# althonos/pyrodigal

Hardware: AMD Instinct MI355X
Metric: Mbp/sec gene-called (meta mode) (higher is better)
Workload: dtype f64; 1 GPU; 100000x20kbp_gc30-70_meta; contigs=100000, bases=2000000000, models=16, contigs_rank0=100000, sub_batch_contigs=6250, contexts_per_gpu=4, genes_all_ranks=2908995, steps_issued=a join of the contexts and a gather per step

## Files before the change

### pyrodigal_amd/csrc/finder.hip

```cpp
#include "pga_internal.h"
#include "pipeline.h"
#include "dpw_core.h"
#include "dev_common.h"

#include <math.h>
#include <stdio.h>
#include <stdlib.h>
#include <string.h>

#include <algorithm>
#include <atomic>
#include <chrono>
#include <condition_variable>
#include <functional>
#include <limits>
#include <map>
#include <memory>
#include <mutex>
#include <new>
#include <thread>
#include <unordered_map>

namespace {

// ... 322 lines not shown
        if (v.strand[ndx] == -1 && next_rev) ig = igm_same_h(v, ndx, next->stop_ndx, w);
        int mi[2] = {-1, -1}; double ms[2] = {0, 0}, mg[2] = {0, 0};
        const int sv_ndx = v.stop_val[ndx];
        constexpr int TWB = 40;
        for (int j0 = ndx - 100; j0 < ndx + 100; j0 += TWB) {
          unsigned long long pass = 0;
#pragma unroll
          for (int q = 0; q < TWB; q++) {
            const int j = j0 + q;
            const int jj = j < 0 ? 0 : (j >= nn ? nn - 1 : j);
            const bool ok = !(is_stop_n(v, jj) | (v.stop_val[jj] != sv_ndx)) && j >= 0 && j < nn && j != ndx;
            pass |= (unsigned long long)ok << q;
          }
          while (pass) {
            const int q = __builtin_ctzll(pass);
            pass &= pass - 1ull;
            const int j = j0 + q;
            double tg = 0.0;
            if (v.strand[j] == 1 && prev_fwd) {
                if (v.ndx[prev->stop_ndx] - v.ndx[j] > maxov) continue;
                tg = igm_same_h(v, prev->stop_ndx, j, w);
            }
            if (v.strand[j] == 1 && prev_rev) { if (v.ndx[prev->start_ndx] - v.ndx[j] >= 0) continue; tg = -0.15 * w; }
            if (v.strand[j] == -1 && next_fwd) { if (v.ndx[j] - v.ndx[next->start_ndx] >= 0) continue; tg = -0.15 * w; }
            if (v.strand[j] == -1 && next_rev) {
                if (v.ndx[j] - v.ndx[next->stop_ndx] > maxov) continue;
                tg = igm_same_h(v, j, next->stop_ndx, w);
            }
            const double cs = v.cscore[j] + v.sscore[j];
            if (mi[0] == -1) { mi[0] = j; ms[0] = cs; mg[0] = tg; }
            else if (cs + tg > ms[0]) { mi[1] = mi[0]; ms[1] = ms[0]; mg[1] = mg[0]; mi[0] = j; ms[0] = cs; mg[0] = tg; }
            else if (mi[1] == -1 || cs + tg > ms[1]) { mi[1] = j; ms[1] = cs; mg[1] = tg; }
          }
        }
        for (int k = 0; k < 2; k++) {
            const int m = mi[k];
            if (m == -1) continue;
            if (v.tscore[m] < v.tscore[ndx] && ms[k] - v.tscore[m] >= sc - v.tscore[ndx] + w && v.rscore[m] > v.rscore[ndx] &&
                v.uscore[m] > v.uscore[ndx] && v.cscore[m] > v.cscore[ndx] && abs(v.ndx[m] - v.ndx[ndx]) > 15) {
                ms[k] += v.tscore[ndx] - v.tscore[m];
            } else if (abs(v.ndx[m] - v.ndx[ndx]) <= 15 && v.rscore[m] + v.tscore[m] > v.rscore[ndx] + v.tscore[ndx] &&
                       v.edge[ndx] == 0 && v.edge[m] == 0) {
                if (v.cscore[ndx] > v.cscore[m]) ms[k] += v.cscore[ndx] - v.cscore[m];
                if (v.uscore[ndx] > v.uscore[m]) ms[k] += v.uscore[ndx] - v.uscore[m];
                if (ig > mg[k]) ms[k] += ig - mg[k];
            } else ms[k] = -1000.0;
        }
        int pick = -1;
        for (int k = 0; k < 2; k++) {
            if (mi[k] == -1) continue;
            if (pick == -1 && ms[k] + mg[k] > sc + ig) pick = k;
            else if (pick >= 0 && ms[k] + mg[k] > ms[pick] + mg[pick]) pick = k;
        }
        if (pick != -1 && v.strand[mi[pick]] == 1) { cur.start_ndx = mi[pick]; cur.begin = v.ndx[mi[pick]] + 1; }
        else if (pick != -1 && v.strand[mi[pick]] == -1) { cur.start_ndx = mi[pick]; cur.end = v.ndx[mi[pick]] + 1; }
    }
}

void tweak_final_starts(const NodeView& v, std::vector<GeneRec>& g, double w, int maxov, int inner_threads = 1, WorkerPool* pool = nullptr) {
    const int ng = (int)g.size();
    if (inner_threads <= 1 || ng < 2048 || pool == nullptr) {
        for (int i = 0; i < ng; i++) tweak_one(v, i > 0 ? &g[i - 1] : nullptr, g[i], i < ng - 1 ? &g[i + 1] : nullptr, w, maxov);
        return;
    }
    const std::vector<GeneRec> orig(g);
    std::atomic<int> next(0);
    auto work = [&]() {
        for (;;) {
            const int i0 = next.fetch_add(256);
            if (i0 >= ng) break;
            for (int i = i0; i < std::min(ng, i0 + 256); i++)
                tweak_one(v, i > 0 ? &orig[i - 1] : nullptr, g[i], i < ng - 1 ? &orig[i + 1] : nullptr, w, maxov);
        }
    };
    pool->run(work, inner_threads);
    for (int i = 1; i < ng; i++) {
        if (g[i - 1].start_ndx == orig[i - 1].start_ndx) continue;
        g[i] = orig[i];
        tweak_one(v, &g[i - 1], g[i], i < ng - 1 ? &orig[i + 1] : nullptr, w, maxov);
    }
}

struct OutArrays;
struct TailDesc {
    int64_t out_off;
    int64_t gene_off;
    int32_t n;
    int32_t mx;
    double  st_wt;
    int64_t fin_off, topo_off;
    int32_t group, _pad;
    int64_t dp_off;
};
struct WinDesc {
    int64_t out_off;
    int64_t dp_off;
    int64_t fin_off;
    int64_t topo_off;
    int32_t n;
    int32_t _pad;
};
struct GcPtrs { const float* p[4]; };
struct OutArrays {
    int32_t* ndx; int32_t* stop_val; uint8_t* type; int8_t* strand; float* gc_cont;
    uint8_t* edge_dp; double* cscore_dp; double* sscore_dp; double* rscore_dp; double* uscore_dp; double* tscore_dp;
    int32_t* star_ptr; int32_t* traceb; int8_t* ov_mark; double* score;
    uint8_t* edge; double* cscore; double* sscore; double* rscore; double* uscore; double* tscore; double* mot_score;
    int32_t* mot_ndx; uint8_t* rbs; uint8_t* mot_len; uint8_t* mot_spacer; uint8_t* mot_spacendx;
    int32_t direct;
    const int32_t* g_ndx[4]; const int32_t* g_stop_val[4]; const uint8_t* g_type[4]; const int8_t* g_strand[4];
    const uint8_t* c_edge; const double* c_cscore; const double* c_rscore; const double* c_uscore; const double* c_tscore;
    const int32_t* c_star_ptr; const double* d_score;
};

__global__ void __launch_bounds__(256)
k_gather_winners(const WinDesc* __restrict__ wd, int n_win, int64_t out_begin, int64_t total, GroupArrays ga, ChainArrays ca,
                 DpBuffers dp, OutArrays o, const int lean ) {
    __shared__ int s_w0;
    const int64_t blk0 = out_begin + (int64_t)blockIdx.x * blockDim.x;
    const int64_t g = blk0 + threadIdx.x;
    int lo = block_search_le([&](const int k) { return wd[k].out_off; }, n_win, blk0, &s_w0);
    if (g >= out_begin + total) return;
    while (lo + 1 < n_win && wd[lo + 1].out_off <= g) lo++;
    const WinDesc w = wd[lo];
    const int i = (int)(g - w.out_off);
    const int64_t t = w.topo_off + i, a = w.dp_off + i, f = w.fin_off + i;
    if (o.direct) { o.sscore_dp[g] = ca.sscore[a]; o.traceb[g] = dp.traceb[a]; o.ov_mark[g] = dp.ov_mark[a]; return; }
    o.ndx[g] = ga.ndx[t]; o.stop_val[g] = ga.stop_val[t]; o.type[g] = ga.type[t]; o.strand[g] = ga.strand[t];
    o.edge_dp[g] = ca.edge[a]; o.cscore_dp[g] = ca.cscore[a]; o.sscore_dp[g] = ca.sscore[a]; o.rscore_dp[g] = ca.rscore[a];
    o.uscore_dp[g] = ca.uscore[a]; o.tscore_dp[g] = ca.tscore[a];
    o.star_ptr[3 * g] = ca.star_ptr[3 * a]; o.star_ptr[3 * g + 1] = ca.star_ptr[3 * a + 1]; o.star_ptr[3 * g + 2] = ca.star_ptr[3 * a + 2];
    o.traceb[g] = dp.traceb[a]; o.ov_mark[g] = dp.ov_mark[a]; o.score[g] = dp.score[a];
    if (lean) return;
    o.gc_cont[g] = ga.gc_cont[t];
    o.edge[g] = ca.edge[f]; o.cscore[g] = ca.cscore[f]; o.sscore[g] = ca.sscore[f]; o.rscore[g] = ca.rscore[f];
    o.uscore[g] = ca.uscore[f]; o.tscore[g] = ca.tscore[f]; o.mot_score[g] = ca.mot_score[f]; o.mot_ndx[g] = ca.mot_ndx[f];
    o.rbs[2 * g] = ca.rbs[2 * f]; o.rbs[2 * g + 1] = ca.rbs[2 * f + 1];
    o.mot_len[g] = ca.mot_len[f]; o.mot_spacer[g] = ca.mot_spacer[f]; o.mot_spacendx[g] = ca.mot_spacendx[f];
}

struct GeneNodeAttr {
    double cscore, sscore, rscore, uscore, tscore, mot_score;
    float gc_cont; int32_t mot_ndx;
    uint8_t edge, rbs0, rbs1, mot_len, mot_spacer, _pad[3];
};
__global__ void __launch_bounds__(256)
k_gather_gene_nodes(const int64_t* __restrict__ idx, int n, OutArrays o, GeneNodeAttr* __restrict__ out) {
    const int t = blockIdx.x * blockDim.x + threadIdx.x;
    if (t >= n) return;
    const int64_t g = idx[t];
    GeneNodeAttr a;
    a.cscore = o.cscore[g]; a.sscore = o.sscore[g]; a.rscore = o.rscore[g]; a.uscore = o.uscore[g]; a.tscore = o.tscore[g];
    a.mot_score = o.mot_score[g]; a.gc_cont = o.gc_cont[g]; a.mot_ndx = o.mot_ndx[g];
    a.edge = o.edge[g]; a.rbs0 = o.rbs[2 * g]; a.rbs1 = o.rbs[2 * g + 1]; a.mot_len = o.mot_len[g]; a.mot_spacer = o.mot_spacer[g];
    a._pad[0] = a._pad[1] = a._pad[2] = 0;
    out[t] = a;
}

__device__ inline NodeView node_view(const TailDesc& d, const OutArrays& o, int32_t* tracef, uint8_t* elim) {
    const int64_t oo = d.out_off;
    if (o.direct) {
        const int64_t t = d.topo_off, a = d.dp_off; const int g = d.group;
        return NodeView{d.n, o.g_ndx[g] + t, o.g_stop_val[g] + t, o.g_type[g] + t, o.g_strand[g] + t, o.c_edge + a,
                        const_cast<double*>(o.c_cscore) + a, o.sscore_dp + oo, o.c_rscore + a, o.c_uscore + a, o.c_tscore + a,
                        o.c_star_ptr + 3 * a, o.traceb + oo, tracef + oo, o.ov_mark + oo, o.d_score + a, elim + oo};
    }
    return NodeView{d.n, o.ndx + oo, o.stop_val + oo, o.type + oo, o.strand + oo, o.edge_dp + oo,
                    o.cscore_dp + oo, o.sscore_dp + oo, o.rscore_dp + oo, o.uscore_dp + oo, o.tscore_dp + oo,
                    o.star_ptr + 3 * oo, o.traceb + oo, tracef + oo, o.ov_mark + oo, o.score + oo, elim + oo};
}

__global__ void __launch_bounds__(64)
k_tail_path(const TailDesc* __restrict__ td, int n_contigs, OutArrays o, int32_t* tracef, uint8_t* elim, int32_t* __restrict__ path,
            GeneRec* __restrict__ genes, int32_t* __restrict__ n_genes) {
    const int i = blockIdx.x * blockDim.x + threadIdx.x;
    if (i >= n_contigs) return;
// ... 159 lines not shown
                  const GeneRec* __restrict__ orig, GeneRec* __restrict__ out, const int32_t* __restrict__ n_genes, int maxov,
                  uint8_t* __restrict__ changed, int32_t* __restrict__ n_changed) {
    const int c = blockIdx.y, lane = threadIdx.x & 63;
    const int g = blockIdx.x * 4 + (threadIdx.x >> 6), ng = n_genes[c];
    if (g >= ng) return;
    const TailDesc d = td[c];
    const NodeView v = node_view(d, o, tracef, elim);
    const GeneRec* base = orig + d.gene_off;
    GeneRec cur = base[g];
    GeneRec prev{}, nxt{};
    if (g > 0) prev = base[g - 1];
    if (g < ng - 1) nxt = base[g + 1];
    tweak_one_wave(v, g > 0 ? &prev : nullptr, cur, g < ng - 1 ? &nxt : nullptr, d.st_wt, maxov, lane);
    if (lane != 0) return;
    out[d.gene_off + g] = cur;
    const bool moved = cur.start_ndx != base[g].start_ndx && v.strand[cur.start_ndx] == -1;
    changed[d.gene_off + g] = moved ? 1 : 0;
    if (moved) atomicAdd(&n_changed[c], 1);
}

#define PGA_FIX_MAXWIN 4096
__global__ void __launch_bounds__(1024)
k_tail_tweak_fixup(const TailDesc* __restrict__ td, int n_contigs, OutArrays o, int32_t* tracef, uint8_t* elim,
                   const GeneRec* __restrict__ orig, const GeneRec* __restrict__ par_all, const int32_t* __restrict__ n_genes, int maxov,
                   const uint8_t* __restrict__ ch0_all, const int32_t* __restrict__ n_changed, GeneRec* __restrict__ fin_all,
                   uint8_t* __restrict__ chf_all) {
    __shared__ uint8_t s_redone[PGA_FIX_MAXWIN];
    const int c = blockIdx.x, lane = threadIdx.x & 63, wave = threadIdx.x >> 6, nwaves = blockDim.x >> 6;
    if (c >= n_contigs) return;
    const TailDesc d = td[c];
    const int ng = n_genes[c];
    const GeneRec* ob = orig + d.gene_off; const GeneRec* par = par_all + d.gene_off; const uint8_t* ch0 = ch0_all + d.gene_off;
    GeneRec* fin = fin_all + d.gene_off; uint8_t* chf = chf_all + d.gene_off;
    for (int g = threadIdx.x; g < ng; g += blockDim.x) { fin[g] = par[g]; chf[g] = ch0[g]; }
    if (n_changed[c] == 0 || ng < 2) return;
    __threadfence_block();
    __syncthreads();
    const NodeView v = node_view(d, o, tracef, elim);
    const int nwin = (ng - 1 + 63) >> 6;
    auto run_window = [&](const int w, const bool assume) -> bool {
        const int g0 = 1 + (w << 6), g1 = min(ng, g0 + 64);
        const int g = g0 + lane;
        if (!assume) {
            if (g < g1) { fin[g] = par[g]; chf[g] = ch0[g]; }
            __builtin_amdgcn_fence(__ATOMIC_RELEASE, "workgroup");
            __builtin_amdgcn_fence(__ATOMIC_ACQUIRE, "workgroup");
        }
        const int pf = g < g1 ? ((lane == 0 && !assume) ? chf[g - 1] : ch0[g - 1]) : 0;
        unsigned long long mask = __ballot(pf != 0);
        bool last = false;
        while (mask) {
            const int k = __builtin_ctzll(mask);
            mask &= mask - 1ull;
            const int gg = g0 + k;
            GeneRec cur = ob[gg];
            const GeneRec prev = (k == 0 && assume) ? par[gg - 1] : fin[gg - 1];
            GeneRec nxt{};
            if (gg < ng - 1) nxt = ob[gg + 1];
            tweak_one_wave(v, &prev, cur, gg < ng - 1 ? &nxt : nullptr, d.st_wt, maxov, lane);
            const int nf = cur.start_ndx != ob[gg].start_ndx && v.strand[cur.start_ndx] == -1;
            if (lane == 0) { fin[gg] = cur; chf[gg] = (uint8_t)nf; }
            __builtin_amdgcn_fence(__ATOMIC_RELEASE, "workgroup");
            __builtin_amdgcn_fence(__ATOMIC_ACQUIRE, "workgroup");
            if (gg + 1 < g1) { if (nf) mask |= 1ull << (k + 1); else mask &= ~(1ull << (k + 1)); }
            if (gg == g1 - 1) last = true;
        }
        return last;
    };
    if (nwin <= PGA_FIX_MAXWIN) {
        for (int w = wave; w < nwin; w += nwaves) { const bool r = run_window(w, true); if (lane == 0) s_redone[w] = r; }
        __threadfence_block();
        __syncthreads();
        if (wave == 0)
            for (int w = 1; w < nwin; w++)
                if (s_redone[w - 1]) { const bool r = run_window(w, false); if (lane == 0) s_redone[w] = r; __builtin_amdgcn_wave_barrier(); }
    } else if (wave == 0) {
        for (int w = 0; w < nwin; w++) run_window(w, false);
    }
}

__global__ void __launch_bounds__(256)
k_emit_genes(const TailDesc* __restrict__ td, int n_contigs, int64_t n_slots, OutArrays o, const GeneRec* __restrict__ fin,
             const int32_t* __restrict__ n_genes, const int64_t* __restrict__ gene_begin, int single, pga_gene* __restrict__ out,
             const int lean, ChainArrays ca, GcPtrs gcs) {
    const int64_t slot = (int64_t)blockIdx.x * blockDim.x + threadIdx.x;
    if (slot >= n_slots) return;
    const int c = contig_of_slot(td, n_contigs, slot);
    const TailDesc d = td[c];
    const int g = (int)(slot - d.gene_off);
    if (g >= n_genes[c]) return;
    const GeneRec gr = fin[slot];
    const int64_t sn = d.out_off + gr.start_ndx, en = d.out_off + gr.stop_ndx;
    pga_gene G;
    memset(&G, 0, sizeof G);
    G.contig = c; G.begin = gr.begin; G.end = gr.end; G.start_ndx = gr.start_ndx; G.stop_ndx = gr.stop_ndx;
    if (o.direct) {
        const int64_t ts = d.topo_off + gr.start_ndx, as = d.dp_off + gr.start_ndx, ae = d.dp_off + gr.stop_ndx;
        const int64_t fs = d.fin_off + gr.start_ndx, fe = d.fin_off + gr.stop_ndx;
        G.strand = o.g_strand[d.group][ts];
        const uint8_t se = single ? o.c_edge[as] : ca.edge[fs], ee = single ? o.c_edge[ae] : ca.edge[fe];
        G.partial_begin = G.strand == 1 ? se : ee; G.partial_end = G.strand == 1 ? ee : se;
        G.start_type = se ? 3 : o.g_type[d.group][ts];
        G.rbs[0] = ca.rbs[2 * fs]; G.rbs[1] = ca.rbs[2 * fs + 1];
        G.mot_len = ca.mot_len[fs]; G.mot_spacer = ca.mot_spacer[fs]; G.mot_ndx = ca.mot_ndx[fs]; G.mot_score = ca.mot_score[fs];
        G.gc_cont = gcs.p[d.group][ts];
        G.cscore = single ? o.c_cscore[as] : ca.cscore[fs]; G.sscore = single ? o.sscore_dp[sn] : ca.sscore[fs];
        G.rscore = single ? o.c_rscore[as] : ca.rscore[fs]; G.uscore = single ? o.c_uscore[as] : ca.uscore[fs];
        G.tscore = single ? o.c_tscore[as] : ca.tscore[fs];
        out[gene_begin[c] + g] = G;
        return;
    }
    G.strand = o.strand[sn];
    if (lean) {
        const int64_t fs = d.fin_off + gr.start_ndx, fe = d.fin_off + gr.stop_ndx;
        const uint8_t se = single ? o.edge_dp[sn] : ca.edge[fs], ee = single ? o.edge_dp[en] : ca.edge[fe];
        G.partial_begin = G.strand == 1 ? se : ee; G.partial_end = G.strand == 1 ? ee : se;
        G.start_type = se ? 3 : o.type[sn];
        G.rbs[0] = ca.rbs[2 * fs]; G.rbs[1] = ca.rbs[2 * fs + 1];
        G.mot_len = ca.mot_len[fs]; G.mot_spacer = ca.mot_spacer[fs]; G.mot_ndx = ca.mot_ndx[fs]; G.mot_score = ca.mot_score[fs];
        G.gc_cont = gcs.p[d.group][d.topo_off + gr.start_ndx];
        G.cscore = single ? o.cscore_dp[sn] : ca.cscore[fs]; G.sscore = single ? o.sscore_dp[sn] : ca.sscore[fs];
        G.rscore = single ? o.rscore_dp[sn] : ca.rscore[fs]; G.uscore = single ? o.uscore_dp[sn] : ca.uscore[fs];
        G.tscore = single ? o.tscore_dp[sn] : ca.tscore[fs];
        out[gene_begin[c] + g] = G;
        return;
    }
    const uint8_t se = single ? o.edge_dp[sn] : o.edge[sn], ee = single ? o.edge_dp[en] : o.edge[en];
    G.partial_begin = G.strand == 1 ? se : ee; G.partial_end = G.strand == 1 ? ee : se;
    G.start_type = se ? 3 : o.type[sn];
    G.rbs[0] = o.rbs[2 * sn]; G.rbs[1] = o.rbs[2 * sn + 1];
    G.mot_len = o.mot_len[sn]; G.mot_spacer = o.mot_spacer[sn]; G.mot_ndx = o.mot_ndx[sn]; G.mot_score = o.mot_score[sn];
    G.gc_cont = o.gc_cont[sn];
    G.cscore = single ? o.cscore_dp[sn] : o.cscore[sn]; G.sscore = single ? o.sscore_dp[sn] : o.sscore[sn];
    G.rscore = single ? o.rscore_dp[sn] : o.rscore[sn]; G.uscore = single ? o.uscore_dp[sn] : o.uscore[sn];
    G.tscore = single ? o.tscore_dp[sn] : o.tscore[sn];
    out[gene_begin[c] + g] = G;
}

__global__ void __launch_bounds__(256)
k_cover_genes(const pga_gene* __restrict__ genes, int64_t n_genes, const ContigDesc* __restrict__ ct, int n_contigs, uint32_t* __restrict__ bits) {
    const int64_t g = (int64_t)blockIdx.x * 4 + (threadIdx.x >> 6);
    const int lane = threadIdx.x & 63;
    if (g >= n_genes) return;
    const int c = genes[g].contig;
    if (c < 0 || c >= n_contigs) return;
    const int32_t b = max(genes[g].begin, 1), e = min(genes[g].end, ct[c].len);
    if (b > e) return;
    const int64_t b0 = ct[c].base + b - 1, b1 = ct[c].base + e - 1;
    const int64_t w0 = b0 >> 5, w1 = b1 >> 5;
    for (int64_t w = w0 + lane; w <= w1; w += 64) {
        uint32_t m = 0xffffffffu;
        if (w == w0) m &= 0xffffffffu << (b0 & 31);
        if (w == w1) m &= 0xffffffffu >> (31 - (b1 & 31));
        atomicOr(&bits[w], m);
    }
}

__global__ void __launch_bounds__(256)
k_count_cover(const uint32_t* __restrict__ bits, const ContigDesc* __restrict__ ct, int64_t* __restrict__ coding) {
    __shared__ int64_t part[4];
    const int c = blockIdx.x;
    const int64_t lo = ct[c].base, len = ct[c].len;
    int64_t n = 0;
    if (len > 0) {
        const int64_t hi = lo + len - 1, w0 = lo >> 5, w1 = hi >> 5;
        for (int64_t w = w0 + threadIdx.x; w <= w1; w += blockDim.x) {
            uint32_t m = bits[w];
            if (w == w0) m &= 0xffffffffu << (lo & 31);
            if (w == w1) m &= 0xffffffffu >> (31 - (hi & 31));
            n += __popc(m);
        }
    }
    for (int d = 32; d > 0; d >>= 1) n += __shfl_down(n, d, 64);
    if ((threadIdx.x & 63) == 0) part[threadIdx.x >> 6] = n;
    __syncthreads();
    if (threadIdx.x == 0) coding[c] = part[0] + part[1] + part[2] + part[3];
}

#include "tail.inl"

struct ResultOwner {
    pga_result pub;
    std::vector<pga_contig_result> contigs;
    std::vector<pga_gene> genes;
    pga_gene* pin_genes = nullptr; size_t pin_cap = 0, pin_n = 0;
    std::vector<pga_nodes> nodes;
    std::vector<int32_t> mask_off, masks;
    bool has_masks = false;
// ... 478 lines not shown
        return PGA_EINVAL;
    }
    const int32_t n_contigs = batch->n;
    if (!c->finder) { int rc0 = pga_finder_models_changed(c); if (rc0) return rc0; }
    const bool meta_run = pp->meta && stage == 0;
    const bool use_sets = meta_run && !batch->sets.empty();
    const bool per_contig = model_of_contig != nullptr && !pp->meta && stage != PGA_STAGE_EXTRACT && stage != PGA_STAGE_SEQUENCE;
    const bool per_contig_tt = tt_of_contig != nullptr && stage == PGA_STAGE_EXTRACT;
    if (c->n_models <= 0 && !meta_run && stage != PGA_STAGE_EXTRACT && stage != PGA_STAGE_SEQUENCE) { c->err = "pga_find_genes: no model loaded (call pga_set_models first)"; return PGA_EINVAL; }
    const pga_params P = *pp;
    const bool mask_union = batch->mask_case != 0 || !batch->regions.empty();
    if ((P.mask || batch->mask_case) && P.min_mask < 0) { c->err = "pga_find_genes: min_mask must be positive"; return PGA_EINVAL; }
    if (!P.closed && P.min_edge_gene > 0 && P.min_edge_gene < 4) {
        c->err = "pga_find_genes: min_edge_gene below 4 is not supported with open ends";
        return PGA_EINVAL;
    }
    if (P.min_gene <= 0 || P.min_edge_gene <= 0 || P.max_overlap < 0 || P.max_overlap > P.min_gene) {
        c->err = "pga_find_genes: invalid min_gene / min_edge_gene / max_overlap";
        return PGA_EINVAL;
    }
    HT(c, hipSetDevice(c->device));
    FinderState* f = c->finder;
    hipStream_t st = c->stream;
    const bool multi = per_contig || per_contig_tt;
    std::vector<int> cgrp, gtt;
    if (per_contig) {
        gtt = f->group_tt;
        for (int i = 0; i < n_contigs; i++) cgrp.push_back(f->model_group[model_of_contig[i]]);
    } else if (per_contig_tt) {
        for (int i = 0; i < n_contigs; i++) {
            int g = (int)(std::find(gtt.begin(), gtt.end(), tt_of_contig[i]) - gtt.begin());
            if (g == (int)gtt.size()) gtt.push_back(tt_of_contig[i]);
            cgrp.push_back(g);
        }
    }
    const int NC = n_contigs, NM = c->n_models, NG = meta_run ? (int)f->group_tt.size() : (multi ? std::max(1, (int)gtt.size()) : 1);
    if (NG > 4) { c->err = "pga_find_genes: more than 4 distinct translation tables loaded"; return PGA_EINVAL; }
    if (const char* fault = getenv("PGA_FAULT_CONTIG_LEN")) {
        const long fl = atol(fault);
        for (int i = 0; i < NC; i++) if ((long)batch->ct[i].len == fl) { c->err = "pga_find_genes: fault injected by PGA_FAULT_CONTIG_LEN"; return PGA_EDEVICE; }
    }

    std::vector<int32_t> set_of;
    int NS = 0;
    if (use_sets) {
        set_of.resize((size_t)NC);
        std::unordered_map<int32_t, int32_t> dense;
        for (int i = 0; i < NC; i++) {
            const int32_t lab = batch->sets[(size_t)i];
            if (lab < 0) { set_of[(size_t)i] = NS++; continue; }
            auto it = dense.find(lab);
            if (it == dense.end()) it = dense.emplace(lab, NS++).first;
            set_of[(size_t)i] = it->second;
        }
        c->set_model.assign((size_t)NC, -1);
        c->set_score.assign((size_t)NC, std::numeric_limits<double>::quiet_NaN());
        c->model_scores.assign((size_t)NC * (size_t)NM, std::numeric_limits<double>::quiet_NaN());
        c->model_scores_nm = NM;
    }

    ResultOwner* R = new (std::nothrow) ResultOwner();
    if (!R) return PGA_ENOMEM;
    struct Guard { ResultOwner* r; ~Guard() { delete r; } } guard{R};
    R->contigs.assign(NC, pga_contig_result{-1, 0, 0, 0, 0, 0.0, 0.0});
    R->mask_off.assign(NC + 1, 0);
    R->has_masks = P.mask || mask_union;
    memset(&R->pub, 0, sizeof R->pub);
    R->pub.n_contigs = NC;

    const std::vector<ContigDesc>& ct = batch->ct;
    const int64_t total = batch->total;
    StageTimer tm;

    if (NC > 0 && total > 0) {
        const char* d_seq = batch->d_seq;
        DEVBUF(d_dig, uint8_t, "d_dig", total + 16);
        DEVBUF(d_ct, ContigDesc, "d_ct", NC + 1);
        const size_t xa_cnt = 4, xa_cbase = xa_cnt + 2 * (size_t)NC, xa_sbase = xa_cbase + (size_t)NG * (NC + 1), xa_en = xa_sbase + (size_t)NG * (NC + 1);
        const size_t xa_words = xa_en + ((size_t)NG * NC + 3) / 4 + 1;
        DEVBUF(d_xa, int32_t, "d_extract_info", xa_words);
        PINBUF(h_xa, int32_t, "h_extract_info", xa_words);
        int32_t* const d_st_overflow = d_xa; int32_t* const h_st_overflow = h_xa;
        int32_t* const d_cnt = d_xa + xa_cnt; int32_t* const h_cnt = h_xa + xa_cnt;
        const int64_t gc_blocks = pga_gc_blocks(total);
        DEVBUF(d_p16, int32_t, "d_gc_p16", total / 16 + 2);
        DEVBUF(d_gc_bsum, int32_t, "d_gc_bsum", gc_blocks + 1);
        DEVBUF(d_gc_boff, int32_t, "d_gc_boff", gc_blocks + 1);
        int32_t* const d_cbase = d_xa + xa_cbase; int32_t* const h_cbase = h_xa + xa_cbase;
        DEVBUF(d_tile_first, int32_t, "d_tile_first", (size_t)6 * batch->n_tiles);
        DEVBUF(d_tile_last, int32_t, "d_tile_last", (size_t)6 * batch->n_tiles);
        DEVBUF(d_tile_count, int32_t, "d_tile_count", (size_t)NG * (batch->n_tiles + 1));
        DEVBUF(d_tile_off, int32_t, "d_tile_off", (size_t)NG * (batch->n_tiles + 1));
        DEVBUF(d_tile_scount, int32_t, "d_tile_scount", (size_t)NG * (batch->n_tiles + 1));
        DEVBUF(d_tile_soff, int32_t, "d_tile_soff", (size_t)NG * (batch->n_tiles + 1));
        int32_t* const d_sbase = d_xa + xa_sbase; int32_t* const h_sbase = h_xa + xa_sbase;
        uint8_t* const d_enabled = (uint8_t*)(d_xa + xa_en); uint8_t* const h_enabled = (uint8_t*)(h_xa + xa_en);

        GroupArrays ga[4];
        for (int g = 0; g < NG; g++) {
            char nm[32];
#define GBUF(field, type, count) { snprintf(nm, sizeof nm, #field "%d", g); void* p__; int rc__ = ensure_dev(c, nm, sizeof(type) * (size_t)(count) + 64, &p__); if (rc__) return rc__; ga[g].field = (type*)p__; }
            GBUF(df, uint8_t, total + 16)
            GBUF(c16, int32_t, (size_t)batch->n_tiles * 192 + 2)
            ga[g].tile0 = batch->d_tile0;
            ga[g].ndx = nullptr; ga[g].stop_val = nullptr; ga[g].type = nullptr; ga[g].strand = nullptr; ga[g].edge0 = nullptr; ga[g].gc_cont = nullptr;
        }

        HT(c, hipEventRecord(f->e_start, st));
        HT(c, hipMemcpyAsync(d_ct, ct.data(), sizeof(ContigDesc) * (NC + 1), hipMemcpyHostToDevice, st));
        HT(c, hipMemsetAsync(d_xa, 0, sizeof(int32_t) * xa_cbase, st));
        pga_launch_digitize(d_seq, d_dig, total, d_ct, NC, d_cnt, d_cnt + NC, st);
        pga_launch_gc_prefix(d_dig, total, d_gc_bsum, d_gc_boff, d_p16, st);
        MaskList masks{nullptr, nullptr};
        int32_t* h_moff = nullptr; const int2* d_union_iv = nullptr;
        if (mask_union) {
            const int64_t per_source = total / std::max(1, P.min_mask) + NC + 1;
            const int64_t most = std::min<int64_t>((P.mask ? per_source : 0) + (batch->mask_case ? per_source : 0) + (int64_t)batch->regions.size(),
                                                   total / 2 + NC + 1);
            const int cap = (int)std::min<int64_t>(most, (int64_t)1 << 28);
            DEVBUF(d_bits, uint32_t, "d_mask_bits", 2 * pga_mask_words(total) + 2);
            DEVBUF(d_mcounts, int32_t, "d_mask_counts", 4 * (pga_mask_waves(total) + 1));
            DEVBUF(d_moff, int32_t, "d_mask_off", NC + 2);
            DEVBUF(d_miv, int2, "d_mask_iv", cap + 1);
            PINBUF(h_moff_, int32_t, "h_mask_off", NC + 2);
            pga_launch_mask_union(d_dig, d_seq, total, d_ct, NC, batch->d_tiles, batch->n_tiles, P.mask, batch->mask_case, P.min_mask, batch->d_regions,
                                  (int)batch->regions.size(), d_bits, d_mcounts, d_moff, d_miv, cap, st);
            HT(c, hipMemcpyAsync(h_moff_, d_moff, sizeof(int32_t) * (NC + 1), hipMemcpyDeviceToHost, st));
            h_moff = h_moff_; d_union_iv = d_miv;
            masks = MaskList{d_moff, d_miv};
        } else if (P.mask) {
            const int cap = (int)std::min<int64_t>(total / std::max(1, P.min_mask) + NC + 1, (int64_t)1 << 28);
            DEVBUF(d_runs, MaskRun, "d_mask_runs", cap + 1);
            DEVBUF(d_nruns, int32_t, "d_mask_count", 4);
            DEVBUF(d_moff, int32_t, "d_mask_off", NC + 2);
            DEVBUF(d_miv, int2, "d_mask_iv", cap + 1);
            pga_launch_find_masks(d_dig, d_ct, NC, batch->d_tiles, batch->n_tiles, P.min_mask, d_runs, d_nruns, cap, st);
            int32_t nruns = 0;
            HT(c, hipMemcpyAsync(&nruns, d_nruns, 4, hipMemcpyDeviceToHost, st));
            HT(c, hipStreamSynchronize(st));
            nruns = std::min(nruns, cap);
            std::vector<MaskRun> runs((size_t)nruns);
            if (nruns > 0) HT(c, hipMemcpy(runs.data(), d_runs, sizeof(MaskRun) * nruns, hipMemcpyDeviceToHost));
            std::sort(runs.begin(), runs.end(), [](const MaskRun& a, const MaskRun& b) { return a.contig != b.contig ? a.contig < b.contig : a.begin < b.begin; });
            std::vector<int32_t> moff(NC + 1, 0);
            std::vector<int2> miv((size_t)nruns + 1);
            for (int k = 0; k < nruns; k++) { moff[runs[k].contig + 1]++; miv[k] = make_int2(runs[k].begin, runs[k].end); }
            for (int i = 0; i < NC; i++) moff[i + 1] += moff[i];
            R->mask_off = moff;
            R->masks.resize(2 * (size_t)nruns);
            for (int k = 0; k < nruns; k++) { R->masks[2 * k] = runs[k].begin; R->masks[2 * k + 1] = runs[k].end; }
            HT(c, hipMemcpy(d_moff, moff.data(), sizeof(int32_t) * (NC + 1), hipMemcpyHostToDevice));
            if (nruns > 0) HT(c, hipMemcpy(d_miv, miv.data(), sizeof(int2) * nruns, hipMemcpyHostToDevice));
            masks = MaskList{d_moff, d_miv};
        }
        if (stage == PGA_STAGE_SEQUENCE) {
            HT(c, hipMemcpyAsync(h_cnt, d_cnt, sizeof(int32_t) * 2 * (size_t)NC, hipMemcpyDeviceToHost, st));
            HT(c, hipGetLastError());
            HT(c, hipStreamSynchronize(st));
            for (int i = 0; i < NC; i++) {
                R->contigs[i].gc = ct[i].len > 0 ? (double)h_cnt[i] / (double)ct[i].len : 0.0;
                R->contigs[i].n_unknown = h_cnt[NC + i];
            }
            if (h_moff) { const int rc = fetch_mask_union(c, R, h_moff, d_union_iv, NC); if (rc) return rc; }
            return publish(R, guard.r, P, out);
        }
        if (meta_run && NM > 0 && use_sets) {
            DEVBUF(d_set_of, int32_t, "d_set_of", 3 * (size_t)NC + 1);
            HT(c, hipMemcpyAsync(d_set_of, set_of.data(), sizeof(int32_t) * (size_t)NC, hipMemcpyHostToDevice, st));
            pga_launch_group_enable_sets(d_ct, NC, d_cnt, d_set_of, d_set_of + NC, f->d_model_gc, f->d_model_grp, NM, NG, d_enabled, st);
        } else if (meta_run && NM > 0) {
            pga_launch_group_enable(d_ct, NC, d_cnt, f->d_model_gc, f->d_model_grp, NM, NG, d_enabled, st);
        }
        if (multi) {
            for (int g = 0; g < NG; g++) for (int i = 0; i < NC; i++) h_enabled[(size_t)g * NC + i] = cgrp[i] == g;
            HT(c, hipMemcpyAsync(d_enabled, h_enabled, (size_t)NG * NC, hipMemcpyHostToDevice, st));
        }
        if (getenv("PGA_STAGE_FULL")) f->stage_full = true;
        bool stage_full = f->stage_full;
        c->extract_passes = 0;
        for (;;) {
            const bool half = !stage_full;
            const int shift = half ? std::max(1, std::min(8, getenv("PGA_STAGE_SHIFT") ? atoi(getenv("PGA_STAGE_SHIFT")) : 1)) : 0;
            const int64_t st_slots = half ? (total >> shift) + (int64_t)PGA_STAGE_SLACK * batch->n_tiles + 8 : 2 * total + 2;
            for (int g = 0; g < NG; g++) {
                char nm[32];
                GBUF(st_ndx, int32_t, st_slots) GBUF(st_sv, int32_t, st_slots) GBUF(st_info, uint8_t, st_slots)
                ga[g].st_half = shift; ga[g].st_overflow = d_st_overflow;
            }
            if (c->extract_passes > 0) HT(c, hipMemsetAsync(d_st_overflow, 0, sizeof(int32_t), st));
            for (int g = 0; g < NG; g++) {
                const int tt = meta_run ? f->group_tt[g] : multi ? gtt[g] : (stage == PGA_STAGE_EXTRACT ? tt_override : c->models[0].trans_table);
                pga_launch_extract(d_dig, total, d_ct, NC, tt, P, ga[g], batch->d_tiles, batch->n_tiles, batch->d_tile0, d_tile_first, d_tile_last,
                                   d_tile_count + (size_t)g * (batch->n_tiles + 1), d_tile_off + (size_t)g * (batch->n_tiles + 1), d_cbase + (size_t)g * (NC + 1),
                                   d_tile_scount + (size_t)g * (batch->n_tiles + 1), d_tile_soff + (size_t)g * (batch->n_tiles + 1), d_sbase + (size_t)g * (NC + 1),
                                   masks, st, ((meta_run && NM > 0) || multi) ? d_enabled + (size_t)g * NC : nullptr);
            }
            HT(c, hipMemcpyAsync(h_xa, d_xa, sizeof(int32_t) * xa_words, hipMemcpyDeviceToHost, st));
            HT(c, hipGetLastError());
            HT(c, hipStreamSynchronize(st));
            c->extract_passes++;
            if (!half || h_st_overflow[0] == 0) break;
            stage_full = true;
            if (!getenv("PGA_STAGE_SHIFT")) f->stage_full = true;
        }
        if (h_moff) { const int rc = fetch_mask_union(c, R, h_moff, d_union_iv, NC); if (rc) return rc; }

        tm.mark("extract+sync");
        int64_t group_nodes[4] = {0, 0, 0, 0};
        for (int g = 0; g < NG; g++) {
            char nm[32];
            group_nodes[g] = h_cbase[(size_t)g * (NC + 1) + NC];
            const int64_t n = group_nodes[g] + 1;
            GBUF(ndx, int32_t, n) GBUF(stop_val, int32_t, n) GBUF(type, uint8_t, n) GBUF(strand, int8_t, n) GBUF(edge0, uint8_t, n) GBUF(gc_cont, float, n) GBUF(contig_of, int32_t, n)
            GBUF(stop_list, int32_t, (int64_t)h_sbase[(size_t)g * (NC + 1) + NC] + 1)
            GBUF(start_list, int32_t, group_nodes[g] - (int64_t)h_sbase[(size_t)g * (NC + 1) + NC] + 1)
            GBUF(ovl_topo, uint32_t, (int64_t)h_sbase[(size_t)g * (NC + 1) + NC] + 1)
            GBUF(srank, int32_t, n + 4)
        }
        for (int g = 0; g < NG; g++) {
            pga_launch_place(d_ct, batch->d_tiles, batch->n_tiles, d_tile_off + (size_t)g * (batch->n_tiles + 1),
                             d_tile_soff + (size_t)g * (batch->n_tiles + 1), ga[g], st);
            pga_launch_orf_gc(d_ct, NC, d_dig, d_p16, ga[g], (int)group_nodes[g], d_cbase + (size_t)g * (NC + 1), st);
        }
        std::vector<std::vector<ChainDesc>> gch(NG);
        std::vector<double> mgc((size_t)NM); std::vector<int> mtt((size_t)NM);
        for (int m = 0; m < NM; m++) { mgc[m] = c->models[m].gc; mtt[m] = c->models[m].trans_table; }
        for (int g = 0; g < NG; g++) gch[g].reserve(meta_run ? (size_t)NC * 6 : (size_t)NC);
        std::vector<double> set_gc;
        if (use_sets) {
            std::vector<int64_t> sum((size_t)2 * NS, 0);
            for (int i = 0; i < NC; i++) { sum[2 * (size_t)set_of[i]] += h_cnt[i]; sum[2 * (size_t)set_of[i] + 1] += ct[i].len; }
            set_gc.resize((size_t)NS);
            for (int s = 0; s < NS; s++) set_gc[(size_t)s] = sum[2 * (size_t)s + 1] > 0 ? (double)sum[2 * (size_t)s] / (double)sum[2 * (size_t)s + 1] : 0.0;
        }
        for (int i = 0; i < NC; i++) {
            const int L = ct[i].len;
            double gc = L > 0 ? (double)h_cnt[i] / (double)L : 0.0;
            R->contigs[i].gc = gc;
            R->contigs[i].n_unknown = h_cnt[NC + i];
            if (!meta_run) {
                const int m = per_contig ? model_of_contig[i] : 0, g = multi ? cgrp[i] : 0;
                const int32_t* cb = h_cbase + (size_t)g * (NC + 1);
                ChainDesc ch{0, cb[i], cb[i + 1] - cb[i], m, i, 1};
                ch.group = g;
                gch[g].push_back(ch);
                continue;
            }
            if (use_sets) gc = set_gc[(size_t)set_of[i]];
            const double low = fmin(0.65, 0.88495 * gc - 0.0102337), high = fmax(0.35, 0.86596 * gc + 0.1131991);
            int tt_prev = -1;
            for (int m = 0; m < NM; m++) {
                if (mgc[m] < low || mgc[m] > high) continue;
                const int g = f->model_group[m];
                if (!h_enabled[(size_t)g * NC + i]) { c->err = "pga_find_genes: host and device disagree on a GC window"; return PGA_EDEVICE; }
                const int32_t* cb = h_cbase + (size_t)g * (NC + 1);
                ChainDesc ch{0, cb[i], cb[i + 1] - cb[i], m, i, mtt[m] != tt_prev ? 1 : 0};
                ch.group = g;
                tt_prev = mtt[m];
                gch[g].push_back(ch);
            }
        }
        std::vector<ChainDesc> chains;
        { size_t tot = 0; for (int g = 0; g < NG; g++) tot += gch[g].size(); chains.reserve(tot); }
        std::vector<int> g_c0(NG + 1, 0);
        std::vector<int64_t> g_n0(NG + 1, 0);
        int64_t tot_chain_nodes = 0, tot_chain_stops = 0;
        std::vector<int64_t> g_s0(NG + 1, 0);
        for (int g = 0; g < NG; g++) {
            g_c0[g] = (int)chains.size(); g_n0[g] = tot_chain_nodes;
            for (ChainDesc& ch : gch[g]) {
                ch.off = tot_chain_nodes; tot_chain_nodes += ch.n;
                ch.soff = tot_chain_stops;
                const int32_t* sb = h_sbase + (size_t)ch.group * (NC + 1);
                tot_chain_stops += sb[ch.contig + 1] - sb[ch.contig];
                chains.push_back(ch);
            }
            g_s0[g + 1] = tot_chain_stops;
        }
        g_c0[NG] = (int)chains.size(); g_n0[NG] = tot_chain_nodes;
        const int NCH = (int)chains.size();
        R->pub.node_passes = tot_chain_nodes;
        R->pub.n_chains = NCH;
        int64_t max_rescore = 0;
        if (meta_run) for (int g = 0; g < NG; g++) max_rescore += h_cbase[(size_t)g * (NC + 1) + NC];
        const int64_t chain_cap = tot_chain_nodes + max_rescore + 64;

        ChainArrays ca;
        {
            DEVBUF(a0, double, "ca_cscore", chain_cap) DEVBUF(a1, double, "ca_sscore", chain_cap) DEVBUF(a2, double, "ca_rscore", chain_cap)
            DEVBUF(a3, double, "ca_uscore", chain_cap) DEVBUF(a4, double, "ca_tscore", chain_cap) DEVBUF(a5, double, "ca_mot_score", chain_cap)
            DEVBUF(a6, int32_t, "ca_star_ptr", 3 * chain_cap) DEVBUF(a7, int32_t, "ca_mot_ndx", chain_cap) DEVBUF(a8, uint8_t, "ca_rbs", 2 * chain_cap)
            DEVBUF(a9, uint8_t, "ca_edge", chain_cap) DEVBUF(a10, uint8_t, "ca_mot_len", chain_cap) DEVBUF(a11, uint8_t, "ca_mot_spacer", chain_cap)
            DEVBUF(a12, uint8_t, "ca_mot_spacendx", chain_cap)
            int64_t max_contig_nodes = 0;
            for (int g = 0; g < NG; g++) for (int i = 0; i < NC; i++)
                max_contig_nodes = std::max<int64_t>(max_contig_nodes, h_cbase[(size_t)g * (NC + 1) + i + 1] - h_cbase[(size_t)g * (NC + 1) + i]);
            DEVBUF(a13, double, "ca_cscore_raw", chain_cap + max_contig_nodes + 64)
            ca = ChainArrays{a0, a1, a2, a3, a4, a5, a13, a6, a7, a8, a9, a10, a11, a12, a13 + chain_cap};
        }
        DpSegPlan seg_plan;
        const bool use_wave = stage == 0 && pga_dp_use_wave(NCH);
        bool seg_wave = false;
        if (stage == 0 && !use_wave && pga_dpw_use_sched() && !getenv("PGA_DP_KERNEL")) {
            int64_t cand = 0;
            const int min_chain = std::max(256, getenv("PGA_DP_SEG_MIN") ? atoi(getenv("PGA_DP_SEG_MIN")) : 16384);
            for (int k = 0; k < NCH; k++) if (chains[(size_t)k].n >= min_chain) cand += chains[(size_t)k].n;
            const char* e = getenv("PGA_DP_SEG_WAVE");
            const char* m = getenv("PGA_DP_SEG_WAVE_MIN");
            seg_wave = e ? atoi(e) != 0 : cand >= (m ? atoll(m) : 2500000ll);
        }
        bool wave_prep = use_wave || seg_wave;
        bool use_sched = wave_prep && pga_dpw_use_sched();
        std::vector<int32_t> h_bbase;
        if (use_sched) {
            h_bbase.resize((size_t)NG * (NC + 1));
            for (int g = 0; g < NG; g++) {
                const int32_t* cb = h_cbase + (size_t)g * (NC + 1);
                int32_t* bb = h_bbase.data() + (size_t)g * (NC + 1);
                bb[0] = 0;
                for (int i = 0; i < NC; i++) bb[i + 1] = bb[i] + ((cb[i + 1] - cb[i] + 63) >> 6);
            }
            for (ChainDesc& ch : chains) ch.sched_b0 = h_bbase[(size_t)ch.group * (NC + 1) + ch.contig];
        }
        int max_batches[4] = {0, 0, 0, 0};
        if (use_sched) for (int g = 0; g < NG; g++) for (int i = 0; i < NC; i++)
            max_batches[g] = std::max(max_batches[g], h_bbase[(size_t)g * (NC + 1) + i + 1] - h_bbase[(size_t)g * (NC + 1) + i]);
        bool segmented = stage == 0 && !use_wave && pga_dp_plan(chains.data(), NCH, tot_chain_nodes, seg_plan, seg_wave);
        if (seg_wave && !segmented) { seg_wave = false; wave_prep = use_wave; use_sched = false; h_bbase.clear(); }
        const bool lean_gather = !P.want_nodes && !(getenv("PGA_TAIL") && strcmp(getenv("PGA_TAIL"), "host") == 0) && !getenv("PGA_FULL_GATHER");
        const bool direct_gather = lean_gather && !getenv("PGA_GATHER_ALL_DP");
        const int64_t dp_cap = tot_chain_nodes + seg_plan.extra + 1;
        const int64_t dp_slots = NCH + (int64_t)seg_plan.segs.size() + 1;
        const int64_t tree_cap = use_wave ? 1 : (seg_wave ? tot_chain_nodes + 1 : dp_cap);
        DpBuffers dp;
        {
            DEVBUF(b0, DpSrc, "dp_src", tree_cap) DEVBUF(b1, DpTgt, "dp_tgt", tree_cap)
            DEVBUF(b2, double, "dp_score", dp_cap) DEVBUF(b3, int32_t, "dp_traceb", dp_cap)
            DEVBUF(b4, int32_t, "dp_tbn", dp_cap) DEVBUF(b5, int8_t, "dp_ov", dp_cap)
            DEVBUF(b7, double, "dp_chain_results", 2 * dp_slots + 2)
            int32_t* const b6 = (int32_t*)(b7 + dp_slots); int32_t* const b8 = b6 + dp_slots;
            DEVBUF(b9, double, "dp_A", tree_cap) DEVBUF(b10, double, "dp_V0", tree_cap) DEVBUF(b11, double, "dp_V1", tree_cap)
            DEVBUF(b12, double, "dp_V2", tree_cap) DEVBUF(b13, double, "dp_hv", tree_cap) DEVBUF(b14, int32_t, "dp_hi", tree_cap)
            dp = DpBuffers{b0, b1, b2, b3, b4, b5, b6, b7, b8, b9, {b10, b11, b12}, b13, b14, nullptr};
        }
        DpwGroupPtrs wgroups{};
        DpwBuffers wbuf{};
        if (wave_prep) {
            for (int g = 0; g < NG; g++) {
                char nm[32];
                const int64_t n = group_nodes[g] + 1;
#define WBUF(field, type) { snprintf(nm, sizeof nm, "dpw_" #field "%d", g); void* p__; int rc__ = ensure_dev(c, nm, sizeof(type) * (size_t)n + 64, &p__); if (rc__) return rc__; wgroups.g[g].field = (type*)p__; }
                WBUF(kf, uint8_t) WBUF(lo, int32_t) WBUF(q1, int32_t) WBUF(q2, int32_t)
#undef WBUF
                wgroups.g[g].ndx = ga[g].ndx; wgroups.g[g].stop_val = ga[g].stop_val; wgroups.g[g].srank = ga[g].srank;
                if (use_sched) {
                    const int64_t nbat = h_bbase[(size_t)g * (NC + 1) + NC];
                    void* p__; int rc__;
                    snprintf(nm, sizeof nm, "dpw_shdr%d", g); rc__ = ensure_dev(c, nm, sizeof(DpwSchedHdr) * (size_t)(nbat + 1), &p__); if (rc__) return rc__; wgroups.g[g].shdr = (DpwSchedHdr*)p__;
                    snprintf(nm, sizeof nm, "dpw_sent%d", g); rc__ = ensure_dev(c, nm, sizeof(DpwSlot) * (size_t)DPW_SCHED_STRIDE * (size_t)(nbat + 1) + 256, &p__); if (rc__) return rc__; wgroups.g[g].sent = (uint4*)p__;
                    snprintf(nm, sizeof nm, "dpw_scur%d", g); rc__ = ensure_dev(c, nm, 64, &p__); if (rc__) return rc__; wgroups.g[g].scur = (uint32_t*)p__;
                }
            }
            DEVBUF(w0, double, "dpw_cs", dp_cap + 2) DEVBUF(w1, DpwExt, "dpw_ext", tot_chain_stops + 4)       DEVBUF(w2, double, "dpw_sfxv", dp_cap) DEVBUF(w3, int32_t, "dpw_sfxi", dp_cap)
            wbuf = DpwBuffers{w0, w1, w2, w3};
            for (int g = 0; g < NG; g++) {
                if (g_c0[g + 1] - g_c0[g] == 0 || g_n0[g + 1] - g_n0[g] == 0 || stage == PGA_STAGE_EXTRACT) continue;
                int max_nodes_g = 0;
                for (int i = 0; i < NC; i++) max_nodes_g = std::max(max_nodes_g, h_cbase[(size_t)g * (NC + 1) + i + 1] - h_cbase[(size_t)g * (NC + 1) + i]);
                if (g < 4) HT(c, hipEventRecord(f->e_aux[4 * g], st));
                pga_launch_dpw_topo(wgroups.g[g], ga[g].type, ga[g].strand, d_cbase + (size_t)g * (NC + 1), NC, (int)group_nodes[g], st, max_nodes_g);
                if (g < 4) HT(c, hipEventRecord(f->e_aux[4 * g + 1], st));
            }
        }
        DpSegDev seg_dev{};
        if (segmented) {
            DEVBUF(seg_arena, char, "dp_seg_arena", pga_dp_seg_bytes(seg_plan, NCH, tot_chain_nodes));
            HT(c, pga_dp_seg_bind(seg_plan, NCH, tot_chain_nodes, seg_arena, st, &seg_dev));
            if (seg_wave) { seg_dev.wave_groups = &wgroups; seg_dev.wave_buf = &wbuf; }
        }
        int32_t* d_dp_order = nullptr;
        std::vector<int32_t> dp_order;
        if (use_wave && NCH > 1 && !getenv("PGA_DP_NO_ORDER")) {
            std::vector<int32_t> lens((size_t)NCH);
            for (int k = 0; k < NCH; k++) lens[(size_t)k] = chains[k].n;
            dp_order.resize((size_t)NCH);
            pga_dp_start_order(NCH, lens.data(), dp_order.data());
            static std::atomic<int> xcc_of[64];
            int n_xcc = xcc_of[c->device & 63].load();
            if (n_xcc == 0) {
                int v = 0;
                n_xcc = (hipDeviceGetAttribute(&v, hipDeviceAttributeNumberOfXccs, c->device) == hipSuccess && v > 0) ? v : 8;
                xcc_of[c->device & 63].store(n_xcc);
            }
            if (!(getenv("PGA_DP_XCD") && atoi(getenv("PGA_DP_XCD")) == 0) && NCH >= 64 && n_xcc == 8) {
                std::vector<int32_t> key((size_t)NCH), by_xcd((size_t)NCH * 8);
                for (int k = 0; k < NCH; k++) key[(size_t)k] = chains[(size_t)k].group * NC + chains[(size_t)k].contig;
                const int64_t nb = pga_dp_xcd_order(NCH, dp_order.data(), lens.data(), key.data(), NC * NG, by_xcd.data(), (int64_t)by_xcd.size());
                int64_t load[8] = {0, 0, 0, 0, 0, 0, 0, 0}, total = 0, heaviest = 0;
                for (int64_t k = 0; k < nb; k++) if (by_xcd[(size_t)k] >= 0) { load[k & 7] += lens[(size_t)by_xcd[(size_t)k]]; total += lens[(size_t)by_xcd[(size_t)k]]; }
                for (int q = 0; q < 8; q++) heaviest = std::max(heaviest, load[q]);
                if (nb > 0 && heaviest * 8 <= total + total * 3 / 10) { by_xcd.resize((size_t)nb); dp_order.swap(by_xcd); }
            }
        }
        PINBUF(h_maxscore, double, "h_chain_results", 2 * dp_slots + 2);
        int32_t* const h_maxidx = (int32_t*)(h_maxscore + dp_slots); int32_t* const h_ipath = h_maxidx + dp_slots;
        PINBUF(h_scur, uint32_t, "h_dpw_scur", 16);
        std::vector<int64_t> ovl_blk0((size_t)NG + 1, 0);
        for (int g = 0; g < NG; g++) ovl_blk0[(size_t)g + 1] = ovl_blk0[(size_t)g] + (g_s0[g + 1] - g_s0[g] + 255) / 256;
        const size_t pa_conv = 0, pa_cc = (((size_t)NG * NC + 1) + 7) & ~(size_t)7, pa_bb = pa_cc + sizeof(int2) * (size_t)2 * NG * NC,
                     pa_ord = pa_bb + ((sizeof(int32_t) * (h_bbase.size() + 1) + 7) & ~(size_t)7),
                     pa_blk = pa_ord + ((sizeof(int32_t) * (dp_order.size() + 1) + 7) & ~(size_t)7),
                     pa_ch = pa_blk + ((sizeof(int32_t) * ((size_t)ovl_blk0[NG] + 1) + 7) & ~(size_t)7), pa_copy = pa_ch + sizeof(ChainDesc) * (size_t)NCH;
        DEVBUF(d_plan, char, "d_call_plan", pa_copy + sizeof(ChainDesc) * ((size_t)NC + 2));
        PINBUF(h_plan, char, "h_call_plan", pa_copy + 64);
        uint8_t* const d_conv = (uint8_t*)(d_plan + pa_conv);
        int2* const d_cc = (int2*)(d_plan + pa_cc); int2* const h_cc = (int2*)(h_plan + pa_cc);
        int32_t* const d_bbase = use_sched ? (int32_t*)(d_plan + pa_bb) : nullptr;
        if (!dp_order.empty()) d_dp_order = (int32_t*)(d_plan + pa_ord);
        ChainDesc* const d_chains = (ChainDesc*)(d_plan + pa_ch);
        memset(h_plan + pa_conv, 0, pa_cc);
        for (size_t k = 0; k < (size_t)2 * NG * NC; k++) h_cc[k] = make_int2(0, 0);
        for (int k = 0; k < NCH; k++) {
            const int g = chains[k].group;
            int2& e = h_cc[(size_t)g * NC + chains[k].contig];
            if (e.y == 0) e.x = k;
            e.y++;
        }
        if (use_sched && !h_bbase.empty()) memcpy(h_plan + pa_bb, h_bbase.data(), sizeof(int32_t) * h_bbase.size());
        if (!dp_order.empty()) memcpy(h_plan + pa_ord, dp_order.data(), sizeof(int32_t) * dp_order.size());
        if (NCH > 0) memcpy(h_plan + pa_ch, chains.data(), sizeof(ChainDesc) * (size_t)NCH);
        const int32_t* const d_ovl_blk = (const int32_t*)(d_plan + pa_blk);
        {
            int32_t* const h_blk = (int32_t*)(h_plan + pa_blk);
            for (int g = 0; g < NG; g++) {
                int k = g_c0[g];
                const int64_t nb = ovl_blk0[(size_t)g + 1] - ovl_blk0[(size_t)g];
                for (int64_t b = 0; b < nb; b++) {
                    const int64_t p0 = g_s0[g] + 256 * b;
                    while (k + 1 < g_c0[g + 1] && chains[(size_t)k + 1].soff <= p0) k++;
                    h_blk[ovl_blk0[(size_t)g] + b] = k - g_c0[g];
                }
            }
        }
        HT(c, hipMemcpyAsync(d_plan, h_plan, pa_copy, hipMemcpyHostToDevice, st));

        tm.mark("plan+alloc");
        std::vector<int32_t> cs_tk[4], cs_en[4];
        ScoreParams sp{P.closed, P.meta, P.max_overlap, NM, nullptr, nullptr};
        PINBUF(h_conv, uint8_t, "h_conv_flag", (size_t)NG * NC + 1);
        const pga_training* d_models = (const pga_training*)c->d_models_raw;
        for (int g = 0; g < NG; g++) {
            const int nch = g_c0[g + 1] - g_c0[g];
            const int64_t nn = g_n0[g + 1] - g_n0[g];
            if (nch == 0 || nn == 0 || stage == PGA_STAGE_EXTRACT) continue;
            const void* d_cs_tasks = nullptr; const void* d_cs_entries = nullptr; int n_cs_tasks = 0;
            const char* cs_env = getenv("PGA_CS_LDS");
            const char* cs_tn = getenv("PGA_CS_TASK_NODES");
            const int cs_task_nodes = cs_tn && atoi(cs_tn) >= 256 && atoi(cs_tn) <= 8192 ? atoi(cs_tn) : 5120;
            if (!(cs_env && atoi(cs_env) == 0) && !f->gil_stride.empty()) {
                std::vector<int32_t>& tk = cs_tk[g]; std::vector<int32_t>& en = cs_en[g];
                if (pga_cs_tasks(h_cc + (size_t)g * NC, NC, chains.data(), h_cbase + (size_t)g * (NC + 1), f->model_rank.data(), cs_task_nodes, tk, en) && !tk.empty()) {
                    char nm1[32], nm2[32];
                    snprintf(nm1, sizeof nm1, "cs_tasks%d", g); snprintf(nm2, sizeof nm2, "cs_entries%d", g);
                    void* p1; void* p2;
                    { int rc__ = ensure_dev(c, nm1, tk.size() * 4 + 64, &p1); if (rc__) return rc__; }
                    { int rc__ = ensure_dev(c, nm2, en.size() * 4 + 64, &p2); if (rc__) return rc__; }
                    HT(c, hipMemcpyAsync(p1, tk.data(), tk.size() * 4, hipMemcpyHostToDevice, st));
                    HT(c, hipMemcpyAsync(p2, en.data(), en.size() * 4, hipMemcpyHostToDevice, st));
                    d_cs_tasks = p1; d_cs_entries = p2; n_cs_tasks = (int)(tk.size() / 4);
                }
            }
            sp.conv_flag = meta_run ? d_conv + (size_t)g * NC : nullptr;
            StopLaunch sl;
            sl.sbase = d_sbase + (size_t)g * (NC + 1); sl.soff_begin = g_s0[g]; sl.n_pairs = g_s0[g + 1] - g_s0[g];
            sl.n_stops = h_sbase[(size_t)g * (NC + 1) + NC];
            sl.starts_only = stage == 0 && !(getenv("PGA_SS_STARTS_ONLY") && atoi(getenv("PGA_SS_STARTS_ONLY")) == 0);
            sl.n_starts = (int32_t)(group_nodes[g] - sl.n_stops);
            sl.blk_chain = d_ovl_blk + ovl_blk0[(size_t)g];
            if (sl.starts_only && sl.n_starts > 0 && NM > 1 && !(getenv("PGA_SS_MM") && atoi(getenv("PGA_SS_MM")) == 0)) {
                std::vector<int64_t> mm_items;
                sl.mm_tiles = pga_mm_tiles(chains.data() + g_c0[g], nch, h_cbase + (size_t)g * (NC + 1), h_sbase + (size_t)g * (NC + 1), NM, mm_items);
                char nm[32];
                void* p__;
                snprintf(nm, sizeof nm, "ss_rec%d", g);
                { int rc__ = ensure_dev(c, nm, PGA_SS_REC_BYTES * (size_t)sl.n_starts + 64, &p__); if (rc__) return rc__; sl.mm_rec = p__; }
                snprintf(nm, sizeof nm, "ss_mmchain%d", g);
                { int rc__ = ensure_dev(c, nm, PGA_SS_MMCHAIN_BYTES * (size_t)nch + 64, &p__); if (rc__) return rc__; sl.mm_chain = p__; }
                snprintf(nm, sizeof nm, "ss_mmtile%d", g);
                { int rc__ = ensure_dev(c, nm, PGA_SS_MMTILE_BYTES * (size_t)sl.mm_tiles + 64, &p__); if (rc__) return rc__; sl.mm_tile = p__; }
                snprintf(nm, sizeof nm, "ss_mmscratch%d", g);
                { int rc__ = ensure_dev(c, nm, pga_mm_scratch_bytes(NM, nch), &p__); if (rc__) return rc__; sl.mm_scratch = p__; }
            }
            sp.cs_out = nullptr;
            if (wave_prep) {
                sl.topo_q2 = wgroups.g[g].q2; sl.ext = wbuf.ext; sp.cs_out = wbuf.cs;
                if (use_wave) {
                    sl.fill_star_ptr = !(stage == 0 && direct_gather);
                    sp.lean_stops = (stage == 0 && direct_gather && sl.starts_only && !getenv("PGA_SS_FULL_STOPS")) ? 1 : 0;
                }
            }
            pga_launch_score(d_chains + g_c0[g], nch, g_n0[g], nn, d_dig, d_ct, ga[g], d_models, f->d_msc, c->d_model_const, ca, sp,
                             d_chains, d_cc + (size_t)g * NC, d_cbase + (size_t)g * (NC + 1), NC, (int)group_nodes[g], f->d_sd_lut, st, 0,
                             (meta_run || per_contig || n_cs_tasks > 0) ? f->d_gil + f->gil_off[g] : nullptr, (meta_run || per_contig || n_cs_tasks > 0) ? f->gil_stride[g] : 0, f->d_model_rank,
                             d_cs_tasks, n_cs_tasks, d_cs_entries, &sl);
            if (wave_prep && use_sched) {
                if (g < 4) HT(c, hipEventRecord(f->e_aux[4 * g + 2], st));
                pga_launch_dpw_sched(wgroups.g[g], d_cbase + (size_t)g * (NC + 1), d_bbase + (size_t)g * (NC + 1), NC, max_batches[g], st);
                if (g < 4) HT(c, hipEventRecord(f->e_aux[4 * g + 3], st));
                HT(c, hipMemcpyAsync(h_scur + 2 * g, wgroups.g[g].scur, 2 * sizeof(uint32_t), hipMemcpyDeviceToHost, st));
            }
            NodeArrays na{ga[g].ndx, ga[g].stop_val, ga[g].type, ga[g].strand, ca.cscore, ca.sscore, ca.rscore, ca.uscore, ca.star_ptr};
            if (!use_wave && stage == 0) pga_launch_dp_prepare(d_chains + g_c0[g], nch, g_n0[g], nn, na, c->d_model_const, dp, st);
        }
        if (stage != 0) {
            const int64_t nn = tot_chain_nodes;
            PINBUF(hs_i32, int32_t, "hs_i32", 6 * nn + 8);
            PINBUF(hs_f64, double, "hs_f64", 6 * nn + 8);
            PINBUF(hs_u8, uint8_t, "hs_u8", 10 * nn + 8);
            PINBUF(hs_f32, float, "hs_f32", nn + 8);
            const bool scored = stage >= PGA_STAGE_SCORE;
            for (int g = 0; g < NG; g++) {
                const int64_t gn = group_nodes[g], o = g_n0[g];
                if (gn == 0) continue;
                HT(c, hipMemcpyAsync(hs_i32 + o, ga[g].ndx, 4 * gn, hipMemcpyDeviceToHost, st));
                HT(c, hipMemcpyAsync(hs_i32 + nn + o, ga[g].stop_val, 4 * gn, hipMemcpyDeviceToHost, st));
                HT(c, hipMemcpyAsync(hs_u8 + o, ga[g].type, gn, hipMemcpyDeviceToHost, st));
                HT(c, hipMemcpyAsync(hs_u8 + nn + o, ga[g].strand, gn, hipMemcpyDeviceToHost, st));
                if (!scored) HT(c, hipMemcpyAsync(hs_u8 + 2 * nn + o, ga[g].edge0, gn, hipMemcpyDeviceToHost, st));
                if (scored) HT(c, hipMemcpyAsync(hs_f32 + o, ga[g].gc_cont, 4 * gn, hipMemcpyDeviceToHost, st));
            }
            if (nn > 0) {
// ... 315 lines not shown
                ngenes += cr.n_genes;
                if (k < 0) { cr.model = -1; continue; }
                cr.model = chains[k].model; cr.n_nodes = chains[k].n;
                cr.score = P.meta ? 0.0 : (h_ipath[k] >= 0 ? h_maxscore[k] : 0.0);
            }
            R->genes.resize((size_t)ngenes);
            PINBUF(h_gidx, int64_t, "h_gidx", 2 * ngenes + 1);
            PINBUF(h_attr, GeneNodeAttr, "h_attr", 2 * ngenes + 1);
            if (ngenes > 0) {
                DEVBUF(d_gidx, int64_t, "d_gidx", 2 * ngenes + 1);
                DEVBUF(d_attr, GeneNodeAttr, "d_attr", 2 * ngenes + 1);
                for (int i = 0; i < NC; i++) {
                    int64_t gi = R->contigs[i].gene_begin;
                    for (const GeneRec& gr : cg[i]) { h_gidx[2 * gi] = out_off[i] + gr.start_ndx; h_gidx[2 * gi + 1] = out_off[i] + gr.stop_ndx; gi++; }
                }
                HT(c, hipMemcpyAsync(d_gidx, h_gidx, sizeof(int64_t) * 2 * ngenes, hipMemcpyHostToDevice, st));
                hipLaunchKernelGGL(k_gather_gene_nodes, dim3((unsigned)((2 * ngenes + 255) / 256)), dim3(256), 0, st, d_gidx, (int)(2 * ngenes), o, d_attr);
                HT(c, hipMemcpyAsync(h_attr, d_attr, sizeof(GeneNodeAttr) * 2 * ngenes, hipMemcpyDeviceToHost, st));
                HT(c, hipGetLastError());
                HT(c, hipStreamSynchronize(st));
            }
            tm.mark("gene_attrs");
            std::atomic<int> next2(0);
            auto filler = [&]() {
                for (;;) {
                    const int i = next2.fetch_add(1);
                    if (i >= NC) break;
                    const int k = win_chain[i];
                    if (k < 0) continue;
                    const int64_t oo = out_off[i];
                    const bool single = !P.meta;
                    int64_t gi = R->contigs[i].gene_begin;
                    for (const GeneRec& gr : cg[i]) {
                        pga_gene& G = R->genes[(size_t)gi];
                        const GeneNodeAttr& as = h_attr[2 * gi]; const GeneNodeAttr& ae = h_attr[2 * gi + 1];
                        gi++;
                        memset(&G, 0, sizeof G);
                        const int64_t sn = oo + gr.start_ndx, en = oo + gr.stop_ndx;
                        G.contig = i; G.begin = gr.begin; G.end = gr.end; G.start_ndx = gr.start_ndx; G.stop_ndx = gr.stop_ndx;
                        G.strand = h.strand[sn];
                        const uint8_t se = single ? h.edge_dp[sn] : as.edge, ee = single ? h.edge_dp[en] : ae.edge;
                        G.partial_begin = G.strand == 1 ? se : ee; G.partial_end = G.strand == 1 ? ee : se;
                        G.start_type = se ? 3 : h.type[sn];
                        G.rbs[0] = as.rbs0; G.rbs[1] = as.rbs1;
                        G.mot_len = as.mot_len; G.mot_spacer = as.mot_spacer; G.mot_ndx = as.mot_ndx; G.mot_score = as.mot_score;
                        G.gc_cont = as.gc_cont;
                        G.cscore = single ? h.cscore_dp[sn] : as.cscore; G.sscore = single ? h.sscore_dp[sn] : as.sscore;
                        G.rscore = single ? h.rscore_dp[sn] : as.rscore; G.uscore = single ? h.uscore_dp[sn] : as.uscore;
                        G.tscore = single ? h.tscore_dp[sn] : as.tscore;
                    }
                }
            };
            run_parallel(filler);
            if (coding) {
                std::vector<std::pair<int32_t, int32_t>> iv;
                for (int i = 0; i < NC; i++) {
                    iv.clear();
                    const int32_t len = ct[i].len;
                    for (const GeneRec& gr : cg[i]) {
                        const int32_t b = std::max<int32_t>(gr.begin, 1), e = std::min<int32_t>(gr.end, len);
                        if (b <= e) iv.emplace_back(b, e);
                    }
                    std::sort(iv.begin(), iv.end());
                    int64_t n = 0; int32_t hi = 0;
                    for (const auto& x : iv) {
                        if (x.second <= hi) continue;
                        n += x.second - std::max(x.first - 1, hi);
                        hi = x.second;
                    }
                    coding[i] = n;
                }
            }
        } else {
            tm.mark("gather");
            std::vector<TailDesc> tdv(NC);
            int64_t n_slots = 0;
            for (int i = 0; i < NC; i++) {
                const int k = win_chain[i];
                TailDesc& d = tdv[i];
                d.out_off = k >= 0 ? out_off[i] : 0; d.gene_off = n_slots;
                d.n = k >= 0 ? chains[k].n : 0; d.mx = k >= 0 ? h_maxidx[k] : -1;
                d.st_wt = k >= 0 ? c->models[chains[k].model].st_wt : 0.0;
                d.fin_off = k >= 0 ? fin_off[i] : 0; d.topo_off = k >= 0 ? chains[k].topo_off : 0;
                d.group = k >= 0 ? chains[k].group : 0; d._pad = 0;
                d.dp_off = k >= 0 ? chains[k].off : 0;
                n_slots += d.n / 2 + 2;
            }
            DEVBUF(d_td, TailDesc, "d_taildesc", NC + 1);
            DEVBUF(d_tracef, int32_t, "d_tracef", out_nodes + 1);
            DEVBUF(d_elim, uint8_t, "d_elim", out_nodes + 1);
            DEVBUF(d_gene0, GeneRec, "d_gene0", n_slots + 1);
            DEVBUF(d_gene1, GeneRec, "d_gene1", n_slots + 1);
            DEVBUF(d_ngenes, int32_t, "d_ngenes", NC + 1);
            DEVBUF(d_gbegin, int64_t, "d_gbegin", NC + 1);
            PINBUF(h_ngenes, int32_t, "h_ngenes", NC + 1);
            PINBUF(h_gbegin, int64_t, "h_gbegin", NC + 1);
            HT(c, hipMemcpyAsync(d_td, tdv.data(), sizeof(TailDesc) * NC, hipMemcpyHostToDevice, st));
            DEVBUF(d_path, int32_t, "d_path", out_nodes + 1);
            DEVBUF(d_changed, uint8_t, "d_changed", n_slots + 1);
            DEVBUF(d_nchanged, int32_t, "d_nchanged", NC + 1);
            const unsigned init_blocks = (unsigned)std::min<int64_t>(2048, (std::max<int64_t>(out_nodes, NC) + 256) / 256);
            if (!par_tail) {
                hipLaunchKernelGGL(k_tail_init, dim3(init_blocks), dim3(256), 0, st, d_tracef, d_elim, out_nodes, d_nchanged, (int32_t*)nullptr, NC, (int32_t*)nullptr, 0);
                hipLaunchKernelGGL(k_tail_path, dim3((NC + 63) / 64), dim3(64), 0, st, d_td, NC, o, d_tracef, d_elim, d_path, d_gene0, d_ngenes);
            } else {
                std::vector<TpSeg> segs;
                bool tail_inited = false;
                for (int i = 0; i < NC; i++) if (win_chain[i] >= 0 && chains[win_chain[i]].n > 0) segs.push_back(TpSeg{out_off[i], chains[win_chain[i]].n, i});
                std::sort(segs.begin(), segs.end(), [](const TpSeg& a, const TpSeg& b) { return a.off < b.off; });
                if (!segs.empty() && out_nodes > 0) {
                    if (out_nodes >= (1ll << 30)) { c->err = "pga_find_genes: more than 2^30 nodes in the winning chains of one batch"; return PGA_EINVAL; }
                    int levels = 1;
                    while ((1ll << levels) < max_n) levels++;
                    const unsigned nblk = (unsigned)((out_nodes + 255) / 256);
                    const bool tp_steps = getenv("PGA_TP_STEPS") != nullptr;
                    const bool tp_one = max_n <= TP_SMALL_MAX && !tp_steps;
                    const int64_t tpn = tp_one ? 0 : out_nodes;
                    DEVBUF(tp_seg, TpSeg, "tp_seg", segs.size()) DEVBUF(tp_up, int32_t, "tp_up", (size_t)2 * tpn)
                    DEVBUF(tp_mark, uint8_t, "tp_mark", tpn) DEVBUF(tp_slots, int32_t, "tp_slots", tpn)
                    DEVBUF(tp_ins, int32_t, "tp_ins", 2 * tpn) DEVBUF(tp_excl, int32_t, "tp_excl", tpn + 1)
                    DEVBUF(tp_bsum, int32_t, "tp_bsum", nblk + 1) DEVBUF(tp_cnt, int32_t, "tp_cnt", segs.size())
                    HT(c, hipMemcpyAsync(tp_seg, segs.data(), sizeof(TpSeg) * segs.size(), hipMemcpyHostToDevice, st));
                    hipLaunchKernelGGL(k_tail_init, dim3(init_blocks), dim3(256), 0, st, d_tracef, d_elim, out_nodes, d_nchanged, d_ngenes, NC,
                                       tp_one ? (int32_t*)nullptr : tp_cnt, (int)segs.size());
                    tail_inited = true;
                    const TpWork tw{tp_seg, (int)segs.size(), out_nodes, levels, tp_up, tp_mark, tp_slots, tp_ins, tp_excl, tp_bsum, tp_cnt};
                    const dim3 grid(nblk), blk(256);
                    if (tp_one) {
                        const int cap = (int)((max_n + 63) & ~63ll);
                        hipLaunchKernelGGL(k_tp_small, dim3((unsigned)segs.size()), dim3(max_n <= 2048 ? 64 : 256), sizeof(int32_t) * 3 * (size_t)cap, st, tw, d_td, o,
                                           d_tracef, d_elim, d_gene0, d_ngenes, cap);
                    } else {
                    hipLaunchKernelGGL(k_tp_init, grid, blk, 0, st, tw, d_td, o);
                    {
                        const bool j8 = !(getenv("PGA_TP_JUMP8") && atoi(getenv("PGA_TP_JUMP8")) == 0);
                        int k = 0;
                        for (int left = levels; left > 0; k++) {
                            const int32_t* in = tp_up + (size_t)(k & 1) * out_nodes; int32_t* outp = tp_up + (size_t)((k + 1) & 1) * out_nodes;
                            if (j8 && left >= 3) { hipLaunchKernelGGL(k_tp_jump8, grid, blk, 0, st, tw, in, outp); left -= 3; }
                            else { hipLaunchKernelGGL(k_tp_jump, grid, blk, 0, st, tw, in, outp); left -= 1; }
                        }
                    }
                    hipLaunchKernelGGL(k_tp_slots, grid, blk, 0, st, tw, d_td, o);
                    hipLaunchKernelGGL(k_tp_scan1, grid, blk, 0, st, tw);
                    hipLaunchKernelGGL(k_tp_scan2, dim3(1), dim3(1024), 0, st, tw, (int)nblk);
                    hipLaunchKernelGGL(k_tp_scan3, grid, blk, 0, st, tw);
                    hipLaunchKernelGGL(k_tp_fill, grid, blk, 0, st, tw, o, d_path);
                    hipLaunchKernelGGL(k_tp_link, grid, blk, 0, st, tw, o, d_path, d_tracef);
                    hipLaunchKernelGGL(k_tp_elim_a, grid, blk, 0, st, tw, d_td, o, d_path);
                    hipLaunchKernelGGL(k_tp_elim_b, grid, blk, 0, st, tw, d_td, o, d_path, d_elim);
                    if (max_n >= 32768 && segs.size() <= 64 && !getenv("PGA_TP_EXTRACT_ONE")) {
                        const int chunks = (max_n + 1023) / 1024;
                        DEVBUF(tp_xsum, TpChunkSum, "tp_xsum", (size_t)chunks * segs.size() + 1);
                        const dim3 xg((unsigned)chunks, (unsigned)segs.size());
                        hipLaunchKernelGGL(k_tp_extract_sum, xg, dim3(1024), 0, st, tw, d_td, o, d_path, d_elim, tp_xsum, chunks);
                        hipLaunchKernelGGL(k_tp_extract_chunk, xg, dim3(1024), 0, st, tw, d_td, o, d_path, d_elim, (const TpChunkSum*)tp_xsum, chunks, d_gene0,
                                           d_ngenes);
                    } else
                    hipLaunchKernelGGL(k_tp_extract, dim3((unsigned)segs.size()), dim3(max_n >= 32768 ? 1024 : 256), 0, st, tw, d_td, o, d_path, d_elim,
                                       d_gene0, d_ngenes);
                    }
                }
                if (!tail_inited) hipLaunchKernelGGL(k_tail_init, dim3(init_blocks), dim3(256), 0, st, d_tracef, d_elim, out_nodes, d_nchanged, d_ngenes, NC, (int32_t*)nullptr, 0);
            }
            if (max_n >= 32768 && NC <= 1024)
                hipLaunchKernelGGL(k_tail_tweak_wave, dim3((unsigned)((max_n / 2 + 2 + 3) / 4), (unsigned)NC), dim3(256), 0, st, d_td, NC, o, d_tracef,
                                   d_elim, d_gene0, d_gene1, d_ngenes, P.max_overlap, d_changed, d_nchanged);
            else if (NC >= 256 && !getenv("PGA_TWEAK_SLOTS")) {
                DEVBUF(d_gpre, int32_t, "d_gene_prefix", NC + 2);
                hipLaunchKernelGGL(k_gene_prefix, dim3(1), dim3(1024), 0, st, d_ngenes, NC, d_gpre);
                hipLaunchKernelGGL(k_tail_tweak_packed, dim3(1024), dim3(256), 0, st, d_td, NC, o, d_tracef, d_elim, d_gene0, d_gene1, d_ngenes,
                                   P.max_overlap, d_changed, d_nchanged, d_gpre);
            } else
                hipLaunchKernelGGL(k_tail_tweak, dim3((unsigned)((n_slots + 255) / 256)), dim3(256), 0, st, d_td, NC, n_slots, o, d_tracef, d_elim,
                                   d_gene0, d_gene1, d_ngenes, P.max_overlap, d_changed, d_nchanged);
            DEVBUF(d_gene2, GeneRec, "d_gene2", n_slots + 1);
            DEVBUF(d_chfin, uint8_t, "d_chfin", n_slots + 1);
            hipLaunchKernelGGL(k_tail_tweak_fixup, dim3(NC), dim3(max_n >= 32768 ? 1024 : 128), 0, st, d_td, NC, o, d_tracef, d_elim, d_gene0, d_gene1,
                               d_ngenes, P.max_overlap, d_changed, d_nchanged, d_gene2, d_chfin);
            HT(c, hipMemcpyAsync(h_ngenes, d_ngenes, sizeof(int32_t) * NC, hipMemcpyDeviceToHost, st));
            HT(c, hipGetLastError());
            HT(c, hipStreamSynchronize(st));
            tm.mark("tail");
            int64_t ngenes = 0;
            for (int i = 0; i < NC; i++) {
                pga_contig_result& cr = R->contigs[i];
                const int k = win_chain[i];
                h_gbegin[i] = ngenes;
                cr.gene_begin = ngenes; cr.n_genes = h_ngenes[i];
                ngenes += cr.n_genes;
                if (k < 0) { cr.model = -1; continue; }
                cr.model = chains[k].model; cr.n_nodes = chains[k].n;
                cr.score = P.meta ? 0.0 : (h_ipath[k] >= 0 ? h_maxscore[k] : 0.0);
            }
            pga_gene* const genes_out = coding || keep ? nullptr : R->gene_records((size_t)ngenes);
            pga_gene* d_genes = nullptr;
            if (ngenes > 0) {
                DEVBUF(d_genes_out, pga_gene, keep ? keep->buf : "d_genes_out", ngenes + 1);
                d_genes = d_genes_out;
                HT(c, hipMemcpyAsync(d_gbegin, h_gbegin, sizeof(int64_t) * NC, hipMemcpyHostToDevice, st));
                GcPtrs gcs{};
                for (int g = 0; g < NG; g++) gcs.p[g] = ga[g].gc_cont;
                hipLaunchKernelGGL(k_emit_genes, dim3((unsigned)((n_slots + 255) / 256)), dim3(256), 0, st, d_td, NC, n_slots, o, d_gene2, d_ngenes,
                                   d_gbegin, P.meta ? 0 : 1, d_genes, lean_gather ? 1 : 0, ca, gcs);
                if (genes_out) HT(c, hipMemcpyAsync(genes_out, d_genes, sizeof(pga_gene) * (size_t)ngenes, hipMemcpyDeviceToHost, st));
                if (keep) { keep->d_genes = d_genes; keep->n_genes = ngenes; }
            }
            if (coding) {
                const int64_t words = total / 32 + 2;
                DEVBUF(d_cover, uint32_t, "d_cover", words);
                DEVBUF(d_coding, int64_t, "d_coding", NC + 1);
                PINBUF(h_coding, int64_t, "h_coding", NC + 1);
                HT(c, hipMemsetAsync(d_cover, 0, sizeof(uint32_t) * (size_t)words, st));
                if (ngenes > 0)
                    hipLaunchKernelGGL(k_cover_genes, dim3((unsigned)((ngenes + 3) / 4)), dim3(256), 0, st, d_genes, ngenes, d_ct, NC, d_cover);
                hipLaunchKernelGGL(k_count_cover, dim3((unsigned)NC), dim3(256), 0, st, d_cover, d_ct, d_coding);
                HT(c, hipMemcpyAsync(h_coding, d_coding, sizeof(int64_t) * NC, hipMemcpyDeviceToHost, st));
                HT(c, hipGetLastError());
                HT(c, hipStreamSynchronize(st));
                memcpy(coding, h_coding, sizeof(int64_t) * NC);
            }
            if (P.want_nodes == 1 && out_nodes > 0) {
                tracef.resize((size_t)out_nodes + 1); elim.resize((size_t)out_nodes + 1);
                HT(c, hipMemcpyAsync(h.ndx, o.ndx, arena_all, hipMemcpyDeviceToHost, st));
                HT(c, hipMemcpyAsync(tracef.data(), d_tracef, sizeof(int32_t) * (size_t)out_nodes, hipMemcpyDeviceToHost, st));
                HT(c, hipMemcpyAsync(elim.data(), d_elim, (size_t)out_nodes, hipMemcpyDeviceToHost, st));
            }
            HT(c, hipEventRecord(f->e_stop, st));
            HT(c, hipGetLastError());
            HT(c, hipStreamSynchronize(st));
            { float ms = 0; HT(c, hipEventElapsedTime(&ms, f->e_start, f->e_stop)); R->pub.t_total_ms = ms; }
            tm.mark("genes+d2h");

        }
        if (P.want_nodes == 1) {
            R->nodes.resize(NC);
            for (int i = 0; i < NC; i++) {
                pga_nodes& N = R->nodes[i];
                memset(&N, 0, sizeof N);
                const int k = win_chain[i];
                if (k < 0) continue;
                const int n = chains[k].n; const int64_t oo = out_off[i];
                const bool single = !P.meta;
                if (int rc = alloc_nodes(R, N, n)) return rc;
                memcpy(N.ndx, h.ndx + oo, 4 * n); memcpy(N.stop_val, h.stop_val + oo, 4 * n); memcpy(N.type, h.type + oo, n); memcpy(N.strand, h.strand + oo, n);
                memcpy(N.gc_cont, h.gc_cont + oo, 4 * n); memcpy(N.rbs, h.rbs + 2 * oo, 2 * n); memcpy(N.mot_ndx, h.mot_ndx + oo, 4 * n);
                memcpy(N.mot_len, h.mot_len + oo, n); memcpy(N.mot_spacer, h.mot_spacer + oo, n); memcpy(N.mot_spacendx, h.mot_spacendx + oo, n);
                memcpy(N.mot_score, h.mot_score + oo, 8 * n);
                if (single) {
                    memcpy(N.edge, h.edge_dp + oo, n); memcpy(N.cscore, h.cscore_dp + oo, 8 * n); memcpy(N.sscore, h.sscore_dp + oo, 8 * n);
                    memcpy(N.rscore, h.rscore_dp + oo, 8 * n); memcpy(N.uscore, h.uscore_dp + oo, 8 * n); memcpy(N.tscore, h.tscore_dp + oo, 8 * n);
                    memcpy(N.score, h.score + oo, 8 * n); memcpy(N.traceb, h.traceb + oo, 4 * n); memcpy(N.tracef, tracef.data() + oo, 4 * n);
                    memcpy(N.ov_mark, h.ov_mark + oo, n); memcpy(N.elim, elim.data() + oo, n); memcpy(N.star_ptr, h.star_ptr + 3 * oo, 12 * n);
                } else {
                    memcpy(N.edge, h.edge + oo, n); memcpy(N.cscore, h.cscore + oo, 8 * n); memcpy(N.sscore, h.sscore + oo, 8 * n);
                    memcpy(N.rscore, h.rscore + oo, 8 * n); memcpy(N.uscore, h.uscore + oo, 8 * n); memcpy(N.tscore, h.tscore + oo, 8 * n);
                    for (int j = 0; j < n; j++) { N.traceb[j] = -1; N.tracef[j] = -1; N.ov_mark[j] = -1; }
                }
            }
        }
        if (P.want_nodes) {
            DevNodes& D = c->dev_nodes;
            D.off.assign(NC, 0); D.n.assign(NC, 0); D.len.resize(NC);
            for (int i = 0; i < NC; i++) {
                D.len[i] = batch->ct[i].len;
                if (win_chain[i] >= 0) { D.off[i] = out_off[i]; D.n[i] = chains[win_chain[i]].n; }
            }
            D.total = out_nodes;
            const bool single = !P.meta;
            D.a = DevNodeArrays{o.ndx, o.stop_val, o.type, o.strand, o.gc_cont,
                                single ? o.edge_dp : o.edge, single ? o.cscore_dp : o.cscore, single ? o.sscore_dp : o.sscore,
                                single ? o.rscore_dp : o.rscore, single ? o.uscore_dp : o.uscore, single ? o.tscore_dp : o.tscore,
                                o.mot_score, o.mot_ndx, o.rbs, o.mot_len, o.mot_spacer};
            D.batch = batch;
            D.contigs = R->contigs.data();
        }
    }
    tm.mark("results");
    return publish(R, guard.r, P, out);
}

static int find_impl(pga_ctx* c, const pga_batch* batch, const pga_params* pp, const int stage, const int tt_override, pga_result** out,
                     const int32_t* model_of_contig, const int32_t* tt_of_contig) {
    return find_impl_cov(c, batch, pp, stage, tt_override, out, model_of_contig, tt_of_contig, nullptr);
}

#include "train.inl"
// ... 179 lines not shown
```

### pyrodigal_amd/csrc/pipeline.h

```cpp
#pragma once
#include "pga_internal.h"

struct ContigDesc {
    int64_t base;
    int32_t len;
    int32_t _pad;
};

#define PGA_STAGE_SLACK 8
struct TileDesc {
    int32_t contig;
    int32_t start;
};

struct GroupArrays {
    uint8_t* df;
    int32_t* c16; const int32_t* tile0 = nullptr;
    int32_t* st_ndx; int32_t* st_sv;
    uint8_t* st_info;
    int32_t st_half = 0; int32_t* st_overflow = nullptr;
    int32_t* stop_list;
    int32_t* start_list = nullptr;
    uint32_t* ovl_topo;
    int32_t* srank = nullptr;
    int32_t* ndx; int32_t* stop_val; uint8_t* type; int8_t* strand; uint8_t* edge0; float* gc_cont;
    int32_t* contig_of = nullptr;
};

struct ChainArrays {
    double* cscore; double* sscore; double* rscore; double* uscore; double* tscore; double* mot_score;
    double* cscore_raw;
    int32_t* star_ptr;
    int32_t* mot_ndx;
    uint8_t* rbs;
    uint8_t* edge;
    uint8_t* mot_len; uint8_t* mot_spacer; uint8_t* mot_spacendx;
    double* cs_sink = nullptr;
};

struct ModelScoreConst {
    double lfac_min, lfac_max;
    double lfac_tab[1001];
};

struct MaskList {
    const int32_t* off;
    const int2* iv;
};
struct MaskRun { int32_t contig, begin, end, _pad; };

struct ScoreParams {
    int32_t closed, is_meta, max_overlap, n_models;
    double* cs_out;
    uint8_t* conv_flag;
    unsigned long long* prof = nullptr;
    int32_t models_per_pass = 512;
    int32_t lean_stops = 0;
};

void pga_launch_digitize(const char* d_seq, uint8_t* d_dig, int64_t total, const ContigDesc* d_ct, int n_contigs,
                         int32_t* d_gc, int32_t* d_unk, hipStream_t st);
int64_t pga_gc_blocks(int64_t total);
void pga_launch_gc_prefix(const uint8_t* d_dig, int64_t total, int32_t* d_block_sum, int32_t* d_block_off, int32_t* d_p16, hipStream_t st);
void pga_launch_extract(const uint8_t* d_dig, int64_t total, const ContigDesc* d_ct, int n_contigs, int tt,
                        const pga_params& p, const GroupArrays& ga, const TileDesc* d_tiles, int n_tiles, const int32_t* d_tile0,
                        int32_t* d_tile_first, int32_t* d_tile_last, int32_t* d_tile_count, int32_t* d_tile_off, int32_t* d_cbase,
                        int32_t* d_tile_scount, int32_t* d_tile_soff, int32_t* d_sbase ,
                        MaskList masks, hipStream_t st,
                        const uint8_t* d_enabled = nullptr );
void pga_launch_place(const ContigDesc* d_ct, const TileDesc* d_tiles, int n_tiles, const int32_t* d_tile_off, const int32_t* d_tile_soff,
                      const GroupArrays& ga, hipStream_t st);
struct StopLaunch {
    const int32_t* sbase = nullptr;
    int64_t soff_begin = 0, n_pairs = 0;
    int32_t n_stops = 0;
    const int32_t* topo_q2 = nullptr; void* ext = nullptr;
    bool fill_star_ptr = true;
    bool starts_only = false; int32_t n_starts = 0;
    const int32_t* blk_chain = nullptr;
    void* mm_rec = nullptr;
    void* mm_chain = nullptr;
    void* mm_tile = nullptr;
    void* mm_scratch = nullptr;
    int32_t mm_tiles = 0;
};
int pga_mm_tile_items();
int32_t pga_mm_tiles(const ChainDesc* h_chains, int n_chains, const int32_t* h_cbase, const int32_t* h_sbase, int n_models, std::vector<int64_t>& scratch);
size_t pga_mm_scratch_bytes(int n_models, int n_chains);
constexpr size_t PGA_SS_REC_BYTES = 32, PGA_SS_MMCHAIN_BYTES = 32, PGA_SS_MMTILE_BYTES = 16;
void pga_launch_group_enable(const ContigDesc* d_ct, int n_contigs, const int32_t* d_gc_count, const double* d_model_gc,
                             const int32_t* d_model_group, int n_models, int n_groups, uint8_t* d_enabled, hipStream_t st);
void pga_launch_group_enable_sets(const ContigDesc* d_ct, int n_contigs, const int32_t* d_gc_count, const int32_t* d_set_of, int32_t* d_pool,
                                  const double* d_model_gc, const int32_t* d_model_group, int n_models, int n_groups, uint8_t* d_enabled,
                                  hipStream_t st);
void pga_launch_find_masks(const uint8_t* d_dig, const ContigDesc* d_ct, int n_contigs, const TileDesc* d_tiles, int n_tiles, int min_mask,
                           MaskRun* d_runs, int32_t* d_count, int cap, hipStream_t st);
int64_t pga_mask_words(int64_t total);
int64_t pga_mask_waves(int64_t total);
void pga_launch_mask_union(const uint8_t* d_dig, const char* d_seq, int64_t total, const ContigDesc* d_ct, int n_contigs, const TileDesc* d_tiles,
                           int n_tiles, int unknown_runs, int lower_case_runs, int min_mask, const MaskRun* d_regions, int n_regions,
                           uint32_t* d_bits, int32_t* d_counts, int32_t* d_moff, int2* d_miv, int cap, hipStream_t st);
int pga_extract_tile_size();
void pga_launch_orf_gc(const ContigDesc* d_ct, int n_contigs, const uint8_t* d_dig, const int32_t* d_p16, const GroupArrays& ga,
                       int n_nodes_total, const int32_t* d_node_contig_base, hipStream_t st);
void pga_launch_score(const ChainDesc* d_chains, int n_chains, int64_t node_begin, int64_t total, const uint8_t* d_dig,
                      const ContigDesc* d_ct, const GroupArrays& ga, const pga_training* d_models,
                      const ModelScoreConst* d_msc, const ModelConst* d_mc, const ChainArrays& ca, ScoreParams sp,
                      const ChainDesc* d_all_chains , const int2* d_contig_chains ,
                      const int32_t* d_node_contig_base, int n_contigs, int group_nodes, const unsigned* d_sd_lut, hipStream_t st,
                      int reuse_raw_cscore = 0 ,
                      const double* d_gil = nullptr , int il_stride = 0,
                      const int32_t* d_rank = nullptr ,
                      const void* d_cs_tasks = nullptr, int n_cs_tasks = 0, const void* d_cs_entries = nullptr ,
                      const StopLaunch* stops = nullptr);
bool pga_cs_tasks(const int2* h_cc, int n_contigs, const ChainDesc* h_chains, const int32_t* h_cbase, const int32_t* model_rank, int task_nodes,
                  std::vector<int32_t>& tasks, std::vector<int32_t>& entries);
void pga_launch_sd_lut(unsigned* d_lut, hipStream_t st);
```

### pyrodigal_amd/csrc/pipeline.hip

```cpp

#include "pga_internal.h"
#include "pipeline.h"
#include <atomic>
#include "dev_common.h"
#include "dpw_core.h"

namespace {

enum { NA = 0, NG = 1, NC = 2, NT = 3, NN = 6 };

__device__ __forceinline__ int find_contig(const ContigDesc* __restrict__ ct, int n, int64_t g) {
    int lo = 0, hi = n - 1;
    while (lo < hi) { int mid = (lo + hi + 1) >> 1; if (ct[mid].base <= g) lo = mid; else hi = mid - 1; }
    return lo;
}

__device__ __forceinline__ int block_contig(const ContigDesc* __restrict__ ct, int n, int64_t block_first, int64_t g, int* s_slot) {
    int c = block_search_le([&](const int k) { return ct[k].base; }, n, block_first, s_slot);
    while (c + 1 < n && ct[c + 1].base <= g) c++;
    return c;
}
__device__ __forceinline__ int block_chain(const ChainDesc* __restrict__ ch, int n, int64_t block_first, int64_t g, int* s_slot) {
    int c = block_search_le([&](const int k) { return ch[k].off; }, n, block_first, s_slot);
    while (c + 1 < n && ch[c + 1].off <= g) c++;
// ... 1470 lines not shown
        }
    }
    const unsigned lo = even_bits(w.p0), hi = even_bits(w.p0 >> 1);
    const unsigned inr = start >= 31 ? 0xfffffffeu : ((2u << start) - 2u);
    w.isA = ~lo & ~hi & inr; w.isG = lo & ~hi & inr;
    return w;
}

__device__ unsigned sd_hits(const int pat, const int q, const int mm) {
    int match[6], limit, cur = 0;
    unsigned hits = 1u;
    const int start = 20, pos = q;
    limit = min(6, start - 4 - pos);
#pragma unroll
    for (int i = 0; i < 6; i++) {
        match[i] = -10;
        if (i >= limit) continue;
        const bool hit = (pat >> i) & 1;
        if (!mm) { if (hit) match[i] = i % 3 == 0 ? 2 : 3; }
        else match[i] = hit ? (i % 3 == 0 ? 2 : 3) : (i % 3 == 0 ? -3 : -2);
    }
    for (int i = limit; i > (mm ? 4 : 2); i--) {
        for (int j = 0; j < limit + 1 - i; j++) {
            int ctr = -2, mism = 0, flag;
#pragma unroll
            for (int k = 0; k < 6; k++) {
                if (k < j || k >= j + i) continue;
                ctr += match[k];
                if (mm && match[k] < 0) { mism++; if (k <= j + 1 || k >= j + i - 2) ctr -= 10; }
            }
            if (mm ? (mism != 1 || ctr < 6) : (ctr < 6)) continue;
            const int rdis = start - (pos + j + i);
            if (!mm) {
                if (rdis < 5) flag = i < 5 ? 2 : 1;
                else if (rdis < 11) flag = 0;
                else if (rdis < 13) flag = i < 5 ? 1 : 2;
                else if (rdis < 16) flag = 3;
                else continue;
                switch (ctr) {
                    case 6:  cur = flag == 0 ? 13 : flag == 1 ? 6 : flag == 2 ? 1 : 2; break;
                    case 8:  cur = flag == 0 ? 15 : flag == 1 ? 12 : flag == 2 ? 11 : 3; break;
                    case 9:  cur = flag == 0 ? 16 : flag == 1 ? 12 : flag == 2 ? 11 : 3; break;
                    case 11: cur = flag == 0 ? 22 : flag == 1 ? 21 : flag == 2 ? 20 : 10; break;
                    case 12: cur = flag == 0 ? 24 : flag == 1 ? 23 : flag == 2 ? 20 : 10; break;
                    case 14: cur = flag == 0 ? 27 : flag == 1 ? 26 : flag == 2 ? 25 : 10; break;
                    default: cur = 0;
                }
            } else {
                if (rdis < 5) flag = 1;
                else if (rdis < 11) flag = 0;
                else if (rdis < 13) flag = 2;
                else if (rdis < 16) flag = 3;
                else continue;
                switch (ctr) {
                    case 6: cur = flag == 0 ? 9 : flag == 1 ? 5 : flag == 2 ? 4 : 2; break;
                    case 7: cur = flag == 0 ? 14 : flag == 1 ? 8 : flag == 2 ? 7 : 2; break;
                    case 9: cur = flag == 0 ? 19 : flag == 1 ? 18 : flag == 2 ? 17 : 3; break;
                    default: break;
                }
            }
            hits |= 1u << cur;
        }
    }
    return hits;
}
#define PGA_SD_LUT 1920
__global__ void k_sd_lut(unsigned* __restrict__ lut) {
    const int t = blockIdx.x * blockDim.x + threadIdx.x;
    if (t < PGA_SD_LUT) lut[t] = sd_hits(t & 63, (t >> 6) % 15, (t >> 6) / 15);
}
__device__ __forceinline__ int sd_pick(unsigned hits, const double* __restrict__ w) {
    int maxv = 0;
    hits &= ~1u;
    while (hits) {
        const int cur = __builtin_ctz(hits);
        hits &= hits - 1u;
        if (w[cur] < w[maxv]) continue;
        if (w[cur] == w[maxv] && cur < maxv) continue;
        maxv = cur;
    }
    return maxv;
}

struct StartModel {
    double st_wt, no_mot;
    int tt, uses_sd;
    double type_wt[3];
    double rbs_wt[28];
    double ups[32][4];
    double mk0[4][64];
    double mk1[4][256];
};

constexpr int SS_EDGE_SPAN = 12;
constexpr int SS_EDGE_CONTIGS = 4;
constexpr int SS_MASK_WORDS = 8;

__device__ __forceinline__ int2 edge_candidate(const GroupArrays& ga, const int tb, const int nn, const int Lc, const int q, const bool closed) {
    const int j = q < SS_EDGE_SPAN ? q : nn - 2 * SS_EDGE_SPAN + q;
    if (j < 0 || j >= nn || (q >= SS_EDGE_SPAN && j < SS_EDGE_SPAN)) return make_int2(0, 0);
    const int svj = ga.stop_val[tb + j], ej = ga.edge0[tb + j], ty = ga.type[tb + j], x = ga.ndx[tb + j], sj = ga.strand[tb + j];
    const bool cv = !closed && ty != PGA_T_STOP && !ej && ((x <= 2 && sj == 1) || (x >= Lc - 3 && sj == -1));
    return make_int2(svj, 4 | (ej ? 1 : 0) | (cv ? 2 : 0));
}

template <int OCC>
__global__ void __launch_bounds__(256, OCC)
k_score_starts(const ChainDesc* __restrict__ chains, const int2* __restrict__ contig_chains,
               const int32_t* __restrict__ node_contig_base, int n_contigs, int n_nodes,
               const uint8_t* __restrict__ dig, const ContigDesc* __restrict__ ct, GroupArrays ga,
               const pga_training* __restrict__ models, ChainArrays ca, ScoreParams sp, const unsigned* __restrict__ sd_lut,
               const int32_t* __restrict__ start_list , const int n_items) {
    __shared__ unsigned long long s_present[SS_MASK_WORDS];
    __shared__ unsigned s_lut[PGA_SD_LUT];
    __shared__ int2 s_edge[SS_EDGE_CONTIGS][2 * SS_EDGE_SPAN];
    __shared__ StartModel SMB[2];
    unsigned long long* __restrict__ prof = sp.prof;
    unsigned long long tp = prof ? __builtin_readcyclecounter() : 0;
    auto mark = [&](const int slot, const bool conv = false) {
        if (!prof) return;
        if (conv) {
#pragma unroll
            for (int m = 32; m >= 1; m >>= 1) { const unsigned long long o = __shfl_xor(tp, m, 64); tp = o > tp ? o : tp; }
        }
        const unsigned long long now = __builtin_readcyclecounter();
        if ((int)(threadIdx.x & 63) == __builtin_ctzll(__ballot(1))) atomicAdd(&prof[slot], now - tp);
        tp = now;
    };
    const int tid = threadIdx.x;
    const int blk0 = blockIdx.x * blockDim.x;
    const bool listed = start_list != nullptr;
    const int n_work = listed ? n_items : n_nodes;
    const bool in_range = blk0 + tid < n_work;
    const int t = listed ? start_list[min(blk0 + tid, n_work - 1)] : blk0 + tid;
    const bool closed = sp.closed != 0, is_meta = sp.is_meta != 0;
    if (tid < SS_MASK_WORDS) s_present[tid] = 0ull;
    const int c0 = ga.contig_of[listed ? start_list[blk0] : blk0];
    const int c = in_range ? ga.contig_of[t] : c0;
    const int2 cc = in_range ? contig_chains[c] : make_int2(0, 0);
    const bool has = in_range && cc.y > 0;
    if (!__syncthreads_or(has) && !listed) return;
    for (int k = tid; k < PGA_SD_LUT; k += blockDim.x) s_lut[k] = sd_lut[k];
    int64_t ch_off = 0, ch_raw = -1; int ch_model = 0x7fffffff, ch_first = 0;
    auto fetch_chain = [&](const int k) { const ChainDesc* __restrict__ q = &chains[k]; ch_off = q->off; ch_model = q->model; ch_first = q->first; ch_raw = q->raw_off; };
    if (has) fetch_chain(cc.x);
    const int tbase = node_contig_base[c];
    const int i = t - tbase, n = has ? node_contig_base[c + 1] - tbase : 1;
    const int type = has ? ga.type[t] : PGA_T_STOP;
    const int e0 = has ? ga.edge0[t] : 0;
    const bool is_start = has && type != PGA_T_STOP;
    const int c_prev = __shfl_up(c, 1, 64);
    const bool enters = has && (listed ? ((tid & 63) == 0 || c != c_prev) : (tid == 0 || i == 0));
    auto enter_models = [&](const int mb) {
        if (!enters) return;
        for (int m = 0; m < cc.y; m++) {
            const int rel = chains[cc.x + m].model - mb;
            if (rel >= 0 && rel < sp.models_per_pass) atomicOr(&s_present[rel >> 6], 1ull << (rel & 63));
        }
    };
    enter_models(0);
    if (tid < SS_EDGE_CONTIGS * 2 * SS_EDGE_SPAN) {
        const int ec = c0 + tid / (2 * SS_EDGE_SPAN), q = tid % (2 * SS_EDGE_SPAN);
        int2 e = make_int2(0, 0);
        if (ec < n_contigs) { const int tb = node_contig_base[ec]; e = edge_candidate(ga, tb, node_contig_base[ec + 1] - tb, ct[ec].len, q, closed); }
        s_edge[tid / (2 * SS_EDGE_SPAN)][q] = e;
    }
// ... 392 lines not shown
    return (cbase[c + 1] - cbase[c]) - (sbase[c + 1] - sbase[c]);
}
constexpr int SS_CNT_LDS = 2048;
__global__ void __launch_bounds__(256)
k_mm_count(const ChainDesc* __restrict__ chains, int n_chains, const int32_t* __restrict__ cbase, const int32_t* __restrict__ sbase,
           int n_models, unsigned long long* __restrict__ cnt, int2* __restrict__ slot) {
    __shared__ unsigned long long s_cnt[SS_CNT_LDS];
    const int tid = threadIdx.x;
    const int k = blockIdx.x * blockDim.x + tid;
    const bool lds = n_models <= SS_CNT_LDS;
    const int model = k < n_chains ? chains[k].model : 0;
    const int n = k < n_chains ? mm_starts_of(cbase, sbase, chains[k].contig) : 0;
    const unsigned long long one = (1ull << 40) | (unsigned long long)n;
    if (lds) {
        for (int m = tid; m < n_models; m += blockDim.x) s_cnt[m] = 0ull;
        __syncthreads();
    }
    unsigned long long v = 0ull;
    if (n > 0) v = lds ? atomicAdd(&s_cnt[model], one) : atomicAdd(&cnt[(size_t)model * SS_CNT_STRIDE], one);
    if (lds) {
        __syncthreads();
        for (int m = tid; m < n_models; m += blockDim.x) {
            const unsigned long long b = s_cnt[m];
            if (b != 0ull) s_cnt[m] = atomicAdd(&cnt[(size_t)m * SS_CNT_STRIDE], b);
        }
        __syncthreads();
        if (n > 0) v += s_cnt[model];
    }
    if (k < n_chains) slot[k] = n > 0 ? make_int2((int)(v >> 40), (int)(v & SS_ITEM_MASK)) : make_int2(-1, 0);
}
__global__ void __launch_bounds__(256)
k_mm_scan(const unsigned long long* __restrict__ cnt, int n_models, const int tile, int32_t* __restrict__ base) {
    __shared__ int s_part[3][257];
    const int tid = threadIdx.x;
    const int per = (n_models + 255) / 256, m0 = min(tid * per, n_models), m1 = min(m0 + per, n_models);
    int a = 0, b = 0, t = 0;
    for (int m = m0; m < m1; m++) {
        const unsigned long long v = cnt[(size_t)m * SS_CNT_STRIDE];
        const int items = (int)(v & SS_ITEM_MASK);
        a += (int)(v >> 40); b += items; t += (items + tile - 1) / tile;
    }
    s_part[0][tid] = a; s_part[1][tid] = b; s_part[2][tid] = t;
    __syncthreads();
    if (tid < 3) {
        int acc = 0;
        for (int q = 0; q < 256; q++) { const int v = s_part[tid][q]; s_part[tid][q] = acc; acc += v; }
    }
    __syncthreads();
    a = s_part[0][tid]; b = s_part[1][tid]; t = s_part[2][tid];
    for (int m = m0; m < m1; m++) {
        base[m] = a; base[n_models + m] = b; base[2 * n_models + m] = t;
        const unsigned long long v = cnt[(size_t)m * SS_CNT_STRIDE];
        const int items = (int)(v & SS_ITEM_MASK);
        a += (int)(v >> 40); b += items; t += (items + tile - 1) / tile;
    }
}
__global__ void __launch_bounds__(256)
k_mm_place(const ChainDesc* __restrict__ chains, int n_chains, const int32_t* __restrict__ cbase, const int32_t* __restrict__ sbase,
           const ContigDesc* __restrict__ ct, const unsigned long long* __restrict__ cnt, const int2* __restrict__ slot,
           const int32_t* __restrict__ base, int n_models, const int tile, const pga_training* __restrict__ models, SsMmChain* __restrict__ mm,
           SsMmTile* __restrict__ tiles) {
    const int k = blockIdx.x * blockDim.x + threadIdx.x;
    if (k >= n_chains) return;
    const int2 s = slot[k];
    if (s.x < 0) return;
    const ChainDesc& ch = chains[k];
    const int m = ch.model, c = ch.contig;
    const int n = mm_starts_of(cbase, sbase, c);
    const int j = base[m] + s.x, ib = base[n_models + m], tb = base[2 * n_models + m];
    const int items_m = (int)(cnt[(size_t)m * SS_CNT_STRIDE] & SS_ITEM_MASK);
    SsMmChain q;
    q.off = ch.off; q.raw = ch.raw_off >= 0 ? ch.raw_off : ch.off;
    q.item0 = ib + s.y; q.n = n;
    q.rdelta = (cbase[c] - sbase[c]) - q.item0;
    q.len_first = (uint32_t)ct[c].len | (ch.first ? 0x80000000u : 0u);
    mm[j] = q;
    for (int tk = s.y / tile; tk <= (s.y + n - 1) / tile; tk++) {
        const int f = tile * tk, l = min(f + tile, items_m) - 1;
        if (f >= s.y) { tiles[tb + tk].j0 = j; tiles[tb + tk].item0 = ib + f; tiles[tb + tk].model_sd = m | (models[m].uses_sd ? (int)0x80000000u : 0); }
        if (l < s.y + n) tiles[tb + tk].j_last = j;
    }
}

template <int TILE>
__global__ void __launch_bounds__(TILE, 8)
k_score_starts_mm(const SsMmTile* __restrict__ tiles, const SsMmChain* __restrict__ mm, const SsStartRec* __restrict__ rec,
                  const pga_training* __restrict__ models, ChainArrays ca, ScoreParams sp, const unsigned* __restrict__ sd_lut) {
    __shared__ StartModelMm SM;
    __shared__ int32_t s_item0[TILE], s_n[TILE], s_rdelta[TILE];
    __shared__ uint32_t s_lf[TILE];
    __shared__ int64_t s_off[TILE], s_raw[TILE];
    unsigned long long* __restrict__ prof = sp.prof;
    unsigned long long tp = prof ? __builtin_readcyclecounter() : 0;
    auto mark = [&](const int slot) {
        if (!prof) return;
        const unsigned long long now = __builtin_readcyclecounter();
        if ((int)(threadIdx.x & 63) == __builtin_ctzll(__ballot(1))) atomicAdd(&prof[slot], now - tp);
        tp = now;
    };
    const int tid = threadIdx.x;
    const SsMmTile T = tiles[blockIdx.x];
    const int nj = min(T.j_last - T.j0 + 1, TILE);
    const pga_training* __restrict__ tm = &models[T.model_sd & 0x7fffffff];
    const int uses_sd = T.model_sd < 0;
    if (tid == 0) { SM.st_wt = tm->st_wt; SM.no_mot = tm->no_mot; SM.tt = tm->trans_table; SM.uses_sd = uses_sd; }
    else if (tid >= 4 && tid < 7) SM.type_wt[tid - 4] = tm->type_wt[tid - 4];
    else if (tid >= 32 && tid < 60) SM.rbs_wt[tid - 32] = tm->rbs_wt[tid - 32];
    else if (tid >= 128 && tid < 256) (&SM.ups[0][0])[tid - 128] = 0.4 * tm->st_wt * (&tm->ups_comp[0][0])[tid - 128];
    if (uses_sd) {
        for (int k = tid; k < PGA_SD_LUT; k += TILE) SM.lut[k] = sd_lut[k];
    } else {
        if (tid < 256) SM.mot.mk0[tid >> 6][tid & 63] = tm->mot_wt[0][tid >> 6][tid & 63];
#pragma unroll
        for (int e = tid; e < 1024; e += TILE) SM.mot.mk1[e >> 8][e & 255] = tm->mot_wt[1][e >> 8][e & 255];
    }
    if (tid < nj) {
        const SsMmChain C = mm[T.j0 + tid];
        s_item0[tid] = C.item0; s_n[tid] = C.n; s_rdelta[tid] = C.rdelta; s_lf[tid] = C.len_first; s_off[tid] = C.off; s_raw[tid] = C.raw;
    }
    __syncthreads();
    mark(0);
    const int item = T.item0 + tid;
    int lo = 0, hi = nj - 1;
    while (lo < hi) { const int mid = (lo + hi + 1) >> 1; if (s_item0[mid] <= item) lo = mid; else hi = mid - 1; }
    if (item < s_item0[lo] + s_n[lo]) {
    const ulonglong2* const rp = (const ulonglong2*)&rec[item + s_rdelta[lo]];
    const ulonglong2 ra = rp[0], rb = rp[1];
    const int64_t raw = s_raw[lo], g0 = s_off[lo];
    const uint32_t len_first = s_lf[lo];
    const unsigned long long ucodes = ra.x, w1 = ra.y, w2 = rb.x, w3 = rb.y;
    const int i = (int)(unsigned)w3;
    const double cs_raw = ca.cscore_raw[raw + i];
    const int64_t g = g0 + i;
    const int L = (int)(len_first & 0x7fffffffu);
    const bool first = (len_first >> 31) != 0;
    const unsigned long long zm = w1 & ((1ull << 42) - 1ull);
    const int nups = (int)((w1 >> 42) & 63u), start = (int)((w1 >> 48) & 63u), type = (int)((w1 >> 54) & 3u);
    const int strand = ((w1 >> 56) & 1u) ? -1 : 1;
    const bool e0 = (w1 >> 57) & 1u, conv = (w1 >> 58) & 1u, ups_near_edge = (w1 >> 59) & 1u, ups_first = (w1 >> 60) & 1u, ups_later = (w1 >> 61) & 1u;
    const unsigned isA = (unsigned)(w2 & 0xfffffu) << 1, isG = (unsigned)((w2 >> 20) & 0xfffffu) << 1;
    const int stop3 = (int)(w2 >> 40);
    const long orf = (long)(w3 >> 32);
    const bool is_meta = sp.is_meta != 0;
    const double st_wt = SM.st_wt;
    const bool stop_missing = !codon_is_stop(stop3 & 0xff, (stop3 >> 8) & 0xff, (stop3 >> 16) & 0xff, SM.tt);
    const bool edge_in = e0 || (conv && !first);
    mark(1);
    int rbs0 = 0, rbs1 = 0, m_ndx = 0, m_len = 0, m_sp = 0, m_si = 0;
    double m_score = 0.0;
    const bool search_sd = !edge_in && SM.uses_sd, search_mot = !edge_in && !SM.uses_sd;
    auto midx = [&](const int k, const int t2) { return (int)((zm >> (2 * (21 - (18 + k - t2)))) & ((1ull << (2 * (k + 3))) - 1ull)); };
    auto msi = [](const int t2) { return t2 <= 2 ? 3 : (t2 <= 4 ? 2 : (t2 >= 11 ? 1 : 0)); };
    auto upstream = [&]() {
        double v = 0.0;
        unsigned lo32 = (unsigned)ucodes, hi32 = (unsigned)(ucodes >> 32);
        if (nups == 32) {
#pragma unroll
            for (int q = 0; q < 16; q++) { v += SM.ups[q][(lo32 >> (2 * q)) & 3u]; if ((q & 7) == 7) __builtin_amdgcn_sched_barrier(0); }
#pragma unroll
            for (int q = 0; q < 16; q++) { v += SM.ups[16 + q][(hi32 >> (2 * q)) & 3u]; if ((q & 7) == 7) __builtin_amdgcn_sched_barrier(0); }
        } else {
            for (int q = 0; q < nups; q++) v += SM.ups[q][(int)(ucodes >> (2 * q)) & 3];
        }
        return v;
    };
    double u = 0.0;
    if (search_sd) {
        unsigned pats[3] = {0u, 0u, 0u};
#pragma unroll
        for (int q = 0; q < 15; q++) {
            const unsigned a6 = (isA >> (15 - q)) & 63u, g6 = (isG >> (15 - q)) & 63u;
            const unsigned pat = ((a6 >> 5) & 1u) | (((g6 >> 4) & 1u) << 1) | (((g6 >> 3) & 1u) << 2) | (((a6 >> 2) & 1u) << 3) |
                                 (((g6 >> 1) & 1u) << 4) | ((g6 & 1u) << 5);
            pats[q / 5] |= pat << (6 * (q % 5));
        }
#pragma unroll
        for (int q = 0; q < 15; q++) {
            if (start - 20 + q < 0 && strand == 1) continue;
            const unsigned pat = (pats[q / 5] >> (6 * (q % 5))) & 63u;
            const unsigned he = SM.lut[(q << 6) | pat], hm = SM.lut[((15 + q) << 6) | pat];
            if (he > 1u) { const int a = sd_pick(he, SM.rbs_wt); if (a > rbs0) rbs0 = a; }
            if (hm > 1u) { const int b = sd_pick(hm, SM.rbs_wt); if (b > rbs1) rbs1 = b; }
        }
    } else if (search_mot) {
        double bsc = -100.0; int bsp = 0, bsi = 0, blen = 0, bndx = 0;
#pragma unroll 1
        for (int k = 3; k >= 0; k--) {
            const int stride = k == 0 ? 64 : (k == 1 ? 256 : 4096);
            const double* __restrict__ gt = &tm->mot_wt[k][0][0];
            const double* lt = k == 1 ? &SM.mot.mk1[0][0] : &SM.mot.mk0[0][0];
            double scv[13];
            if (k >= 2) {
#pragma unroll
                for (int t2 = 0; t2 < 13; t2++) scv[t2] = 18 + k - t2 > start ? -1000.0 : gt[msi(t2) * stride + midx(k, t2)];
            } else {
#pragma unroll
                for (int t2 = 0; t2 < 13; t2++) scv[t2] = 18 + k - t2 > start ? -1000.0 : lt[msi(t2) * stride + midx(k, t2)];
            }
#pragma unroll
            for (int t2 = 0; t2 < 13; t2++)
                if (scv[t2] > bsc) { bsc = scv[t2]; bsi = msi(t2); bsp = 15 - t2; blen = k + 3; bndx = midx(k, t2); }
        }
        if (bsc == -4.0 || bsc < SM.no_mot + 0.69) { m_score = SM.no_mot; }
        else { m_ndx = bndx; m_len = blen; m_si = bsi; m_sp = bsp & 15; m_score = bsc; }
    }
    if (!edge_in) u = upstream();
    mark(2);
    double edge_gene = 0;
    if (edge_in) edge_gene += 1;
    if (stop_missing) edge_gene += 1;

    double tscore, uscore, rscore, sscore, cscore = cs_raw;
    if (edge_in) {
        tscore = 0.74 * st_wt / edge_gene; uscore = 0.0; rscore = 0.0;
    } else {
        tscore = SM.type_wt[type] * st_wt;
        const double r1 = SM.rbs_wt[rbs0], r2 = SM.rbs_wt[rbs1];
        const double sd = fmax(r1, r2) * st_wt;
        if (SM.uses_sd) rscore = sd;
        else { rscore = st_wt * m_score; if (rscore < sd && SM.no_mot > -0.5) rscore = sd; }
        uscore = u;
        if (ups_near_edge || (first ? ups_first : ups_later)) uscore += -1.00 * st_wt;
    }
    bool edge_now = edge_in;
    if (conv && !edge_in) {
        edge_gene += 1; edge_now = true; tscore = 0.0;
        uscore = 0.74 * st_wt / edge_gene; rscore = 0.0;
    }
    if (!edge_now && edge_gene == 1) uscore -= 0.5 * 0.74 * st_wt;
    if (edge_gene == 0 && orf < 250) {
        const double negf = 250.0 / (float)orf, posf = (float)orf / 250.0;
        rscore *= rscore < 0 ? negf : posf;
        uscore *= uscore < 0 ? negf : posf;
        tscore *= tscore < 0 ? negf : posf;
    }
    if (is_meta && L < 3000 && edge_gene == 0 && (cscore < 5.0 || orf < 120))
        cscore -= 7.5 * fmax(0.0, (3000.0 - L) / 2700.0);
    sscore = tscore + rscore + uscore;
    if (cscore < 0.0) {
        if (edge_gene > 0 && !edge_now) {
            if (!is_meta || L > 1500) sscore -= st_wt; else sscore -= 10.31 - 0.004 * L;
        } else if (is_meta && L < 3000 && edge_now) {
            const double mml = sqrt((double)L) * 5.0;
            if (orf >= mml) { if (cscore >= 0) cscore = -1.0; sscore = 0.0; uscore = 0.0; }
        } else sscore -= 0.5;
    } else if (is_meta && cscore < 5.0 && orf < 120 && sscore < 0.0) sscore -= st_wt;
    mark(3);
    ca.cscore[g] = cscore; ca.sscore[g] = sscore; ca.rscore[g] = rscore; ca.uscore[g] = uscore; ca.tscore[g] = tscore;
    ca.mot_score[g] = m_score; ca.mot_ndx[g] = m_ndx;
    ca.mot_len[g] = (uint8_t)m_len; ca.mot_spacer[g] = (uint8_t)m_sp; ca.mot_spacendx[g] = (uint8_t)m_si;
    ca.rbs[2 * g] = (uint8_t)rbs0; ca.rbs[2 * g + 1] = (uint8_t)rbs1;
    ca.edge[g] = (uint8_t)edge_now;
    if (sp.cs_out != nullptr) sp.cs_out[g] = cscore + sscore;
    mark(4);
    }
}

struct OvlChain {
    const int32_t* __restrict__ ndx; const int32_t* __restrict__ stv; const uint8_t* __restrict__ typ; const int8_t* __restrict__ str;
    const double* __restrict__ cs; const double* __restrict__ ss; const double* __restrict__ rs; const double* __restrict__ us;
    int n;
    const double* __restrict__ css = nullptr;
};
constexpr int OV_SPEC = 16;
__device__ __forceinline__ unsigned overlap_neighbours(const int32_t* __restrict__ ndx, const int32_t* __restrict__ stv, const uint8_t* __restrict__ typ,
                                                       const int8_t* __restrict__ str, const int n, const int i, const int maxov) {
    const int my = ndx[i];
    const bool fwd = str[i] == 1;
    bool ended = false;
    unsigned elig = 0;
    constexpr int OV_NEAR = 10;
#pragma unroll
    for (int k = 0; k < OV_SPEC; k++) {
        if (k == OV_NEAR && ended) break;
        const int j = fwd ? i + 3 - k : i - 3 + k;
        const int jj = min(max(j, 0), n - 1);
        const int nd = ndx[jj], sv = stv[jj], ty = typ[jj], sd = str[jj];
        bool stop_here, ok;
        if (fwd) {
            stop_here = j < 0 || (j < n && nd <= my + 2 && nd + maxov < my);
            ok = j >= 0 && j < n && nd <= my + 2 && sd == 1 && ty != PGA_T_STOP && sv > my;
        } else {
            stop_here = j >= n || (j >= 0 && nd >= my - 2 && nd - maxov > my);
            ok = j >= 0 && j < n && nd >= my - 2 && sd == -1 && ty != PGA_T_STOP && sv < my;
        }
        ended = ended || stop_here;
        if (ok && !ended) {
            elig |= 1u << k;
            if (k < 15 && (fwd ? (my + 2 == nd || my == nd + 1) : (nd + 2 == my || nd == my + 1))) elig |= 0x10000u << k;
        }
    }
    return elig | (ended ? 0x80000000u : 0u);
}

__device__ __forceinline__ void overlapping_starts_of(const OvlChain& C, const int i, const ModelConst* __restrict__ mc, const int maxov,
                                                      int& sp0, int& sp1, int& sp2, const unsigned neighbours) {
    const int32_t* __restrict__ ndx = C.ndx; const int32_t* __restrict__ stv = C.stv;
    const uint8_t* __restrict__ typ = C.typ; const int8_t* __restrict__ str = C.str;
    const double* __restrict__ cs = C.cs; const double* __restrict__ ss = C.ss; const double* __restrict__ rs = C.rs; const double* __restrict__ us = C.us;
    const int n = C.n;
    const int my = ndx[i];
    double best = -100;
    const bool fwd = str[i] == 1;
    const double rs_i = 0.0, us_i = 0.0;
    unsigned elig = neighbours & 0xffffu;
    int js = fwd ? i + 3 - OV_SPEC : i - 3 + OV_SPEC;
    bool more = !(neighbours >> 31);
    for (;;) {
        int j = -1;
        if (elig) {
            const int k = __builtin_ctz(elig);
            elig &= elig - 1u;
            j = fwd ? i + 3 - k : i - 3 + k;
        } else {
            while (more) {
                if (fwd ? js < 0 : js >= n) { more = false; break; }
                const int jq = js;
                js += fwd ? -1 : 1;
                if (jq < 0 || jq >= n) continue;
                const int nq = ndx[jq];
                if (fwd ? nq > my + 2 : nq < my - 2) continue;
                if (fwd ? nq + maxov < my : nq - maxov > my) { more = false; break; }
                if (str[jq] != (fwd ? 1 : -1) || typ[jq] == PGA_T_STOP) continue;
                if (fwd ? stv[jq] <= my : stv[jq] >= my) continue;
                j = jq;
                break;
            }
            if (j < 0) break;
        }
        const int nj = ndx[j];
        const double csj = C.css != nullptr ? C.css[j] : cs[j] + ss[j];
        const bool adj = fwd ? (my + 2 == nj || my == nj + 1) : (nj + 2 == my || nj == my + 1);
        const double rj = adj ? rs[j] : 0.0, uj = adj ? us[j] : 0.0;
        const double v = fwd ? csj + igm_same_dev(my, 1, rs_i, us_i, nj, rj, uj, mc->st_wt, mc->igm)
                             : csj + igm_same_dev(nj, -1, rj, uj, my, rs_i, us_i, mc->st_wt, mc->igm);
        if (v > best) { const int f = nj % 3; if (f == 0) sp0 = j; else if (f == 1) sp1 = j; else sp2 = j; best = v; }
    }
// ... 416 lines not shown
    for (int q = 63; q >= 0; q--) {
        const std::vector<int32_t>& b = bucket[(size_t)q];
        int first = (int)(entries.size() / 4), count = 0, nodes = 0, cuts = 0;
        auto flush = [&]() {
            if (count > 0) { tasks.push_back(q); tasks.push_back(first); tasks.push_back(count); tasks.push_back(0); }
            first += count; count = 0; nodes = 0; cuts = 0;
        };
        for (size_t k = 0; k < b.size(); k += 2) {
            const int nc = h_cbase[b[k] + 1] - h_cbase[b[k]];
            for (int f0 = 0; f0 < nc; f0 += task_nodes) {
                const int piece = std::min(task_nodes, nc - f0);
                if (count > 0 && (nodes + piece > task_nodes || count == CS_TASK_MAX_ENTRIES || (piece != nc && cuts == CS_TASK_MAX_CUTS))) flush();
                entries.push_back(b[k]); entries.push_back(b[k + 1]); entries.push_back(f0); entries.push_back(piece);
                count++; nodes += piece; cuts += piece != nc;
            }
        }
        flush();
    }
    return true;
}

__global__ void __launch_bounds__(256)
k_group_enable(const ContigDesc* __restrict__ ct, int n_contigs, const int32_t* __restrict__ gc_count, const double* __restrict__ model_gc,
               const int32_t* __restrict__ model_group, int n_models, int n_groups, uint8_t* __restrict__ enabled ) {
    const int i = blockIdx.x * blockDim.x + threadIdx.x;
    if (i >= n_contigs) return;
    const int L = ct[i].len;
    const double gc = L > 0 ? (double)gc_count[i] / (double)L : 0.0;
    const double low = fmin(0.65, 0.88495 * gc - 0.0102337), high = fmax(0.35, 0.86596 * gc + 0.1131991);
    unsigned need = 0;
    for (int m = 0; m < n_models; m++) if (!(model_gc[m] < low || model_gc[m] > high)) need |= 1u << model_group[m];
    for (int g = 0; g < n_groups; g++) enabled[(size_t)g * n_contigs + i] = (need >> g) & 1;
}
void pga_launch_group_enable(const ContigDesc* d_ct, int n_contigs, const int32_t* d_gc_count, const double* d_model_gc,
                             const int32_t* d_model_group, int n_models, int n_groups, uint8_t* d_enabled, hipStream_t st) {
    if (n_contigs <= 0) return;
    hipLaunchKernelGGL(k_group_enable, dim3(nblocks(n_contigs, 256)), dim3(256), 0, st, d_ct, n_contigs, d_gc_count, d_model_gc, d_model_group,
                       n_models, n_groups, d_enabled);
}

__global__ void __launch_bounds__(256)
k_set_pool(const ContigDesc* __restrict__ ct, int n_contigs, const int32_t* __restrict__ gc_count, const int32_t* __restrict__ set_of,
           int32_t* __restrict__ pool) {
    const int i = blockIdx.x * blockDim.x + threadIdx.x;
    if (i >= n_contigs) return;
    const int s = set_of[i];
    if (s < 0 || s >= n_contigs) return;
    atomicAdd(pool + 2 * (size_t)s, gc_count[i]);
    atomicAdd(pool + 2 * (size_t)s + 1, (int32_t)ct[i].len);
}
__global__ void __launch_bounds__(256)
k_group_enable_sets(int n_contigs, const int32_t* __restrict__ set_of, const int32_t* __restrict__ pool, const double* __restrict__ model_gc,
                    const int32_t* __restrict__ model_group, int n_models, int n_groups, uint8_t* __restrict__ enabled ) {
    const int i = blockIdx.x * blockDim.x + threadIdx.x;
    if (i >= n_contigs) return;
    const int s = set_of[i];
    const bool ok = s >= 0 && s < n_contigs;
    const int L = ok ? pool[2 * (size_t)s + 1] : 0;
    const double gc = L > 0 ? (double)pool[2 * (size_t)s] / (double)L : 0.0;
    const double low = fmin(0.65, 0.88495 * gc - 0.0102337), high = fmax(0.35, 0.86596 * gc + 0.1131991);
    unsigned need = 0;
    for (int m = 0; m < n_models; m++) if (!(model_gc[m] < low || model_gc[m] > high)) need |= 1u << model_group[m];
    for (int g = 0; g < n_groups; g++) enabled[(size_t)g * n_contigs + i] = (need >> g) & 1;
}
void pga_launch_group_enable_sets(const ContigDesc* d_ct, int n_contigs, const int32_t* d_gc_count, const int32_t* d_set_of, int32_t* d_pool,
                                  const double* d_model_gc, const int32_t* d_model_group, int n_models, int n_groups, uint8_t* d_enabled,
                                  hipStream_t st) {
    if (n_contigs <= 0) return;
    (void)hipMemsetAsync(d_pool, 0, sizeof(int32_t) * 2 * (size_t)n_contigs, st);
    hipLaunchKernelGGL(k_set_pool, dim3(nblocks(n_contigs, 256)), dim3(256), 0, st, d_ct, n_contigs, d_gc_count, d_set_of, d_pool);
    hipLaunchKernelGGL(k_group_enable_sets, dim3(nblocks(n_contigs, 256)), dim3(256), 0, st, n_contigs, d_set_of, d_pool, d_model_gc, d_model_group,
                       n_models, n_groups, d_enabled);
}



void pga_launch_orf_gc(const ContigDesc* d_ct, int n_contigs, const uint8_t* d_dig, const int32_t* d_p16, const GroupArrays& ga,
                       int n_nodes_total, const int32_t* d_node_contig_base, hipStream_t st) {
    if (n_nodes_total <= 0) return;
    hipLaunchKernelGGL(k_orf_gc, dim3(nblocks(n_nodes_total, 256)), dim3(256), 0, st, d_ct, n_contigs, d_dig, d_p16, ga,
                       n_nodes_total, d_node_contig_base);
}

void pga_launch_sd_lut(unsigned* d_lut, hipStream_t st) {
    hipLaunchKernelGGL(k_sd_lut, dim3((PGA_SD_LUT + 255) / 256), dim3(256), 0, st, d_lut);
}

int pga_mm_tile_items() {
    const char* e = getenv("PGA_SS_MM_TILE");
    const int v = e ? atoi(e) : 0;
    return v == 256 || v == 512 || v == 1024 ? v : SS_TILE_DEFAULT;
}
int32_t pga_mm_tiles(const ChainDesc* h_chains, int n_chains, const int32_t* h_cbase, const int32_t* h_sbase, int n_models, std::vector<int64_t>& items) {
    const int tile = pga_mm_tile_items();
    items.assign((size_t)n_models, 0);
    for (int k = 0; k < n_chains; k++) {
        const int c = h_chains[k].contig;
        items[(size_t)h_chains[k].model] += (h_cbase[c + 1] - h_cbase[c]) - (h_sbase[c + 1] - h_sbase[c]);
    }
    int64_t tiles = 0;
    for (int m = 0; m < n_models; m++) tiles += (items[(size_t)m] + tile - 1) / tile;
    return (int32_t)tiles;
}
size_t pga_mm_scratch_bytes(int n_models, int n_chains) {
    return sizeof(unsigned long long) * SS_CNT_STRIDE * (size_t)n_models + sizeof(int32_t) * (((size_t)3 * n_models + 1) & ~(size_t)1) + sizeof(int2) * (size_t)n_chains + 64;
}

void pga_launch_score(const ChainDesc* d_chains, int n_chains, int64_t node_begin, int64_t total, const uint8_t* d_dig,
                      const ContigDesc* d_ct, const GroupArrays& ga, const pga_training* d_models,
                      const ModelScoreConst* d_msc, const ModelConst* d_mc, const ChainArrays& ca, ScoreParams sp,
                      const ChainDesc* d_all_chains, const int2* d_contig_chains, const int32_t* d_node_contig_base, int n_contigs,
                      int group_nodes, const unsigned* d_sd_lut, hipStream_t st, int reuse_raw_cscore, const double* d_gil, int il_stride,
                      const int32_t* d_rank, const void* d_cs_tasks, int n_cs_tasks, const void* d_cs_entries, const StopLaunch* stops) {
    if (total <= 0 || n_chains <= 0) return;
    const dim3 grid(nblocks(total, 256)), blk(256);
    if (group_nodes > 0 && !reuse_raw_cscore && n_cs_tasks > 0) {
        static std::atomic<bool> attr_set[64];
        static std::atomic<unsigned long long*> prof_of[64];
        int dev = 0;
        (void)hipGetDevice(&dev);
        dev &= 63;
        const size_t lds = sizeof(double) * 4096 * 4;
        int cs_wave = CS_WAVE;
        if (const char* e = getenv("PGA_CS_WAVE")) cs_wave = atoi(e) >= 64 ? atoi(e) : CS_WAVE;
        if (!attr_set[dev].load()) {
            hipFuncSetAttribute((const void*)k_coding_score_quads, hipFuncAttributeMaxDynamicSharedMemorySize, (int)lds);
            attr_set[dev].store(true);
        }
        const bool profiling = getenv("PGA_CS_PROFILE") != nullptr;
        unsigned long long* d_prof = prof_of[dev].load();
        if (profiling) {
            if (!d_prof) { (void)hipMalloc((void**)&d_prof, 16 * sizeof(unsigned long long)); prof_of[dev].store(d_prof); }
            (void)hipMemsetAsync(d_prof, 0, 16 * sizeof(unsigned long long), st);
        }
        hipLaunchKernelGGL(k_coding_score_quads, dim3((unsigned)n_cs_tasks), dim3(CS_TASK_THREADS), lds, st, (const CsTask*)d_cs_tasks,
                           (const CsEntry*)d_cs_entries, d_all_chains, d_contig_chains, d_node_contig_base, d_dig, d_ct, ga, d_models, d_msc, ca,
                           d_gil, il_stride, d_rank, cs_wave, profiling ? d_prof : nullptr, (getenv("PGA_CS_QCLASSES") && atoi(getenv("PGA_CS_QCLASSES")) == 4) ? 4 : 3);
        if (profiling) {
            unsigned long long h[16];
            (void)hipStreamSynchronize(st);
            (void)hipMemcpy(h, d_prof, sizeof h, hipMemcpyDeviceToHost);
            fprintf(stderr, "[pga cs-profile] %d tasks (%llu workgroups, %llu batches of 64): wave-cycles  stage %.3g  list %.3g  one-wave ORFs %.3g  "
                            "four-to-a-wave %.3g  64-to-a-wave %.3g (lookup %.3g  first loads %.3g  walk %.3g  penalties %.3g)  end barrier %.3g\n",
                    n_cs_tasks, h[7], h[8], (double)h[0], (double)h[1], (double)h[2], (double)h[3], (double)h[4], (double)h[9], (double)h[10], (double)h[11],
                    (double)h[12], (double)h[5]);
        }
        reuse_raw_cscore = 1;
    }
    if (group_nodes > 0 && !reuse_raw_cscore)
        hipLaunchKernelGGL(k_coding_score, dim3(nblocks(group_nodes, 256)), blk, 0, st, d_all_chains, d_contig_chains, d_node_contig_base,
                           n_contigs, 0, group_nodes, d_dig, d_ct, ga, d_models, d_msc, ca, d_gil, il_stride, d_rank);
    if (group_nodes > 0) {
        if (const char* e = getenv("PGA_SS_MODELS_PER_PASS")) { const int v = atoi(e); if (v >= 1 && v <= 512) sp.models_per_pass = v; }
        static std::atomic<unsigned long long*> ss_prof_of[64];
        const bool ss_profiling = getenv("PGA_SS_PROFILE") != nullptr;
        if (ss_profiling) {
            int dev = 0; (void)hipGetDevice(&dev); dev &= 63;
            unsigned long long* d_prof = ss_prof_of[dev].load();
            if (!d_prof) { (void)hipMalloc((void**)&d_prof, 16 * sizeof(unsigned long long)); ss_prof_of[dev].store(d_prof); }
            (void)hipMemsetAsync(d_prof, 0, 16 * sizeof(unsigned long long), st);
            sp.prof = d_prof;
        }
        const bool listed = stops != nullptr && stops->starts_only && ga.start_list != nullptr;
        const int n_items = listed ? stops->n_starts : group_nodes;
        const bool mm = listed && n_items > 0 && stops->mm_tiles > 0 && stops->mm_rec != nullptr && !(getenv("PGA_SS_MM") && atoi(getenv("PGA_SS_MM")) == 0);
        if (mm) {
            const int nm = sp.n_models;
            unsigned long long* const d_cnt = (unsigned long long*)stops->mm_scratch;
            int32_t* const d_base = (int32_t*)(d_cnt + (size_t)SS_CNT_STRIDE * nm);
            int2* const d_slot = (int2*)(d_base + (((size_t)3 * nm + 1) & ~(size_t)1));
            (void)hipMemsetAsync(d_cnt, 0, sizeof(unsigned long long) * SS_CNT_STRIDE * (size_t)nm, st);
            hipLaunchKernelGGL(k_start_prologue, dim3(nblocks(n_items, 256)), blk, 0, st, d_contig_chains, d_node_contig_base, n_contigs, d_dig, d_ct, ga, sp,
                               (const int32_t*)ga.start_list, n_items, (SsStartRec*)stops->mm_rec);
            hipLaunchKernelGGL(k_mm_count, dim3(nblocks(n_chains, 256)), blk, 0, st, d_chains, n_chains, d_node_contig_base, stops->sbase, nm, d_cnt, d_slot);
            const int tile = pga_mm_tile_items();
            hipLaunchKernelGGL(k_mm_scan, dim3(1), blk, 0, st, (const unsigned long long*)d_cnt, nm, tile, d_base);
            hipLaunchKernelGGL(k_mm_place, dim3(nblocks(n_chains, 256)), blk, 0, st, d_chains, n_chains, d_node_contig_base, stops->sbase, d_ct,
                               (const unsigned long long*)d_cnt, (const int2*)d_slot, (const int32_t*)d_base, nm, tile, d_models, (SsMmChain*)stops->mm_chain, (SsMmTile*)stops->mm_tile);
            const SsMmTile* const d_tl = (const SsMmTile*)stops->mm_tile; const SsMmChain* const d_mc = (const SsMmChain*)stops->mm_chain;
            const SsStartRec* const d_rec = (const SsStartRec*)stops->mm_rec;
            const dim3 grid_mm((unsigned)stops->mm_tiles);
            if (tile == 1024) hipLaunchKernelGGL(k_score_starts_mm<1024>, grid_mm, dim3(1024), 0, st, d_tl, d_mc, d_rec, d_models, ca, sp, d_sd_lut);
            else if (tile == 512) hipLaunchKernelGGL(k_score_starts_mm<512>, grid_mm, dim3(512), 0, st, d_tl, d_mc, d_rec, d_models, ca, sp, d_sd_lut);
            else hipLaunchKernelGGL(k_score_starts_mm<256>, grid_mm, blk, 0, st, d_tl, d_mc, d_rec, d_models, ca, sp, d_sd_lut);
            if (stops->n_stops > 0)
                hipLaunchKernelGGL(k_clear_stops, dim3(nblocks(stops->n_stops, 256)), blk, 0, st, d_all_chains, d_contig_chains, d_node_contig_base, ga, ca, sp,
                                   stops->n_stops);
        } else if (n_items > 0)
            hipLaunchKernelGGL(k_score_starts<4>, dim3(nblocks(n_items, 256)), blk, 0, st, d_all_chains, d_contig_chains, d_node_contig_base, n_contigs,
                               group_nodes, d_dig, d_ct, ga, d_models, ca, sp, d_sd_lut, listed ? (const int32_t*)ga.start_list : (const int32_t*)nullptr, n_items);
        if (ss_profiling && mm) {
            unsigned long long h[16];
            (void)hipStreamSynchronize(st);
            (void)hipMemcpy(h, sp.prof, sizeof h, hipMemcpyDeviceToHost);
            fprintf(stderr, "[pga ss-profile] model-major, %d starts, %d tiles: wave-cycles  stage %.3g  chain + record %.3g  upstream + RBS / motif search %.3g  "
                            "scores %.3g  stores %.3g\n", n_items, stops->mm_tiles, (double)h[0], (double)h[1], (double)h[2], (double)h[3], (double)h[4]);
        } else if (ss_profiling) {
            unsigned long long h[16];
            (void)hipStreamSynchronize(st);
            (void)hipMemcpy(h, sp.prof, sizeof h, hipMemcpyDeviceToHost);
            fprintf(stderr, "[pga ss-profile] %d nodes: wave-cycles  locate %.3g  node + upstream window %.3g  barrier + edge scan %.3g | per model: next model %.3g  "
                            "chain %.3g  upstream + RBS / motif search %.3g  scores %.3g  finish + stores (slot 8) %.3g  stage %.3g  barrier %.3g (slot 7 unused %.3g)\n",
                    group_nodes, (double)h[0], (double)h[1], (double)h[2], (double)h[3], (double)h[4], (double)h[5], (double)h[6], (double)h[8],
                    (double)h[9], (double)h[10], (double)h[7]);
        }
    }
    if (stops != nullptr) {
        if (stops->fill_star_ptr) (void)hipMemsetAsync(ca.star_ptr + 3 * node_begin, 0xff, sizeof(int32_t) * 3 * (size_t)total, st);
        if (stops->n_pairs > 0 && stops->n_stops > 0)
            hipLaunchKernelGGL(k_ovl_topo, dim3(nblocks(stops->n_stops, 256)), blk, 0, st, ga, d_node_contig_base, stops->sbase, n_contigs, stops->n_stops,
                               sp.max_overlap);
        if (stops->n_pairs > 0)
            hipLaunchKernelGGL(k_ovl_stops, dim3(nblocks(stops->n_pairs, 256)), blk, 0, st, d_chains, n_chains, stops->soff_begin, stops->n_pairs, ga,
                               d_node_contig_base, stops->sbase, d_mc, ca, sp.max_overlap, stops->topo_q2, (DpwExt*)stops->ext,
                               stops->ext != nullptr ? (const double*)sp.cs_out : nullptr, getenv("PGA_OVL_SEARCH") ? nullptr : stops->blk_chain);
    } else hipLaunchKernelGGL(k_overlapping_starts, grid, blk, 0, st, d_chains, n_chains, node_begin, total, ga, d_mc, ca, sp.max_overlap);
}
```

Before: 21180 Mbp/s.

## Compute GC content and RBS/motif fields only for final genes

When only genes are wanted, the per-node GC prefix sum, ORF GC computation and gc_cont buffer are skipped. The start-scoring kernel no longer stores RBS/motif fields for every candidate start. A new post-pass kernel recomputes GC content, SD RBS and motif fields only for emitted genes, using 4 lanes per gene. This trades per-node memory traffic and scans for a small recompute over the gene list, but the motif search still runs during scoring for score values and the recomputed fields must match the originals exactly.

```diff
diff --git a/pyrodigal_amd/csrc/finder.hip b/pyrodigal_amd/csrc/finder.hip
--- a/pyrodigal_amd/csrc/finder.hip
+++ b/pyrodigal_amd/csrc/finder.hip
@@ -428,16 +428,6 @@
 }
 
 struct OutArrays;
-struct TailDesc {
-    int64_t out_off;
-    int64_t gene_off;
-    int32_t n;
-    int32_t mx;
-    double  st_wt;
-    int64_t fin_off, topo_off;
-    int32_t group, _pad;
-    int64_t dp_off;
-};
 struct WinDesc {
     int64_t out_off;
     int64_t dp_off;
@@ -763,7 +753,7 @@
 __global__ void __launch_bounds__(256)
 k_emit_genes(const TailDesc* __restrict__ td, int n_contigs, int64_t n_slots, OutArrays o, const GeneRec* __restrict__ fin,
              const int32_t* __restrict__ n_genes, const int64_t* __restrict__ gene_begin, int single, pga_gene* __restrict__ out,
-             const int lean, ChainArrays ca, GcPtrs gcs) {
+             const int lean, ChainArrays ca, GcPtrs gcs, const int gene_only ) {
     const int64_t slot = (int64_t)blockIdx.x * blockDim.x + threadIdx.x;
     if (slot >= n_slots) return;
     const int c = contig_of_slot(td, n_contigs, slot);
@@ -782,9 +772,11 @@
         const uint8_t se = single ? o.c_edge[as] : ca.edge[fs], ee = single ? o.c_edge[ae] : ca.edge[fe];
         G.partial_begin = G.strand == 1 ? se : ee; G.partial_end = G.strand == 1 ? ee : se;
         G.start_type = se ? 3 : o.g_type[d.group][ts];
-        G.rbs[0] = ca.rbs[2 * fs]; G.rbs[1] = ca.rbs[2 * fs + 1];
-        G.mot_len = ca.mot_len[fs]; G.mot_spacer = ca.mot_spacer[fs]; G.mot_ndx = ca.mot_ndx[fs]; G.mot_score = ca.mot_score[fs];
-        G.gc_cont = gcs.p[d.group][ts];
+        if (!gene_only) {
+            G.rbs[0] = ca.rbs[2 * fs]; G.rbs[1] = ca.rbs[2 * fs + 1];
+            G.mot_len = ca.mot_len[fs]; G.mot_spacer = ca.mot_spacer[fs]; G.mot_ndx = ca.mot_ndx[fs]; G.mot_score = ca.mot_score[fs];
+            G.gc_cont = gcs.p[d.group][ts];
+        }
         G.cscore = single ? o.c_cscore[as] : ca.cscore[fs]; G.sscore = single ? o.sscore_dp[sn] : ca.sscore[fs];
         G.rscore = single ? o.c_rscore[as] : ca.rscore[fs]; G.uscore = single ? o.c_uscore[as] : ca.uscore[fs];
         G.tscore = single ? o.c_tscore[as] : ca.tscore[fs];
@@ -1429,10 +1421,17 @@
         PINBUF(h_xa, int32_t, "h_extract_info", xa_words);
         int32_t* const d_st_overflow = d_xa; int32_t* const h_st_overflow = h_xa;
         int32_t* const d_cnt = d_xa + xa_cnt; int32_t* const h_cnt = h_xa + xa_cnt;
-        const int64_t gc_blocks = pga_gc_blocks(total);
-        DEVBUF(d_p16, int32_t, "d_gc_p16", total / 16 + 2);
-        DEVBUF(d_gc_bsum, int32_t, "d_gc_bsum", gc_blocks + 1);
-        DEVBUF(d_gc_boff, int32_t, "d_gc_boff", gc_blocks + 1);
+        const bool lean_gather = !P.want_nodes && !(getenv("PGA_TAIL") && strcmp(getenv("PGA_TAIL"), "host") == 0) && !getenv("PGA_FULL_GATHER");
+        const bool direct_gather = lean_gather && !getenv("PGA_GATHER_ALL_DP");
+        const bool gene_only = stage == 0 && direct_gather && !(getenv("PGA_GENE_FIELDS") && strcmp(getenv("PGA_GENE_FIELDS"), "stored") == 0);
+        int32_t* d_p16 = nullptr; int32_t* d_gc_bsum = nullptr; int32_t* d_gc_boff = nullptr;
+        if (!gene_only) {
+            const int64_t gc_blocks = pga_gc_blocks(total);
+            DEVBUF(p16, int32_t, "d_gc_p16", total / 16 + 2);
+            DEVBUF(bsum, int32_t, "d_gc_bsum", gc_blocks + 1);
+            DEVBUF(boff, int32_t, "d_gc_boff", gc_blocks + 1);
+            d_p16 = p16; d_gc_bsum = bsum; d_gc_boff = boff;
+        }
         int32_t* const d_cbase = d_xa + xa_cbase; int32_t* const h_cbase = h_xa + xa_cbase;
         DEVBUF(d_tile_first, int32_t, "d_tile_first", (size_t)6 * batch->n_tiles);
         DEVBUF(d_tile_last, int32_t, "d_tile_last", (size_t)6 * batch->n_tiles);
@@ -1457,7 +1456,7 @@
         HT(c, hipMemcpyAsync(d_ct, ct.data(), sizeof(ContigDesc) * (NC + 1), hipMemcpyHostToDevice, st));
         HT(c, hipMemsetAsync(d_xa, 0, sizeof(int32_t) * xa_cbase, st));
         pga_launch_digitize(d_seq, d_dig, total, d_ct, NC, d_cnt, d_cnt + NC, st);
-        pga_launch_gc_prefix(d_dig, total, d_gc_bsum, d_gc_boff, d_p16, st);
+        if (!gene_only) pga_launch_gc_prefix(d_dig, total, d_gc_bsum, d_gc_boff, d_p16, st);
         MaskList masks{nullptr, nullptr};
         int32_t* h_moff = nullptr; const int2* d_union_iv = nullptr;
         if (mask_union) {
@@ -1558,7 +1557,8 @@
             char nm[32];
             group_nodes[g] = h_cbase[(size_t)g * (NC + 1) + NC];
             const int64_t n = group_nodes[g] + 1;
-            GBUF(ndx, int32_t, n) GBUF(stop_val, int32_t, n) GBUF(type, uint8_t, n) GBUF(strand, int8_t, n) GBUF(edge0, uint8_t, n) GBUF(gc_cont, float, n) GBUF(contig_of, int32_t, n)
+            GBUF(ndx, int32_t, n) GBUF(stop_val, int32_t, n) GBUF(type, uint8_t, n) GBUF(strand, int8_t, n) GBUF(edge0, uint8_t, n) GBUF(contig_of, int32_t, n)
+            if (!gene_only) GBUF(gc_cont, float, n)
             GBUF(stop_list, int32_t, (int64_t)h_sbase[(size_t)g * (NC + 1) + NC] + 1)
             GBUF(start_list, int32_t, group_nodes[g] - (int64_t)h_sbase[(size_t)g * (NC + 1) + NC] + 1)
             GBUF(ovl_topo, uint32_t, (int64_t)h_sbase[(size_t)g * (NC + 1) + NC] + 1)
@@ -1567,7 +1567,7 @@
         for (int g = 0; g < NG; g++) {
             pga_launch_place(d_ct, batch->d_tiles, batch->n_tiles, d_tile_off + (size_t)g * (batch->n_tiles + 1),
                              d_tile_soff + (size_t)g * (batch->n_tiles + 1), ga[g], st);
-            pga_launch_orf_gc(d_ct, NC, d_dig, d_p16, ga[g], (int)group_nodes[g], d_cbase + (size_t)g * (NC + 1), st);
+            if (!gene_only) pga_launch_orf_gc(d_ct, NC, d_dig, d_p16, ga[g], (int)group_nodes[g], d_cbase + (size_t)g * (NC + 1), st);
         }
         std::vector<std::vector<ChainDesc>> gch(NG);
         std::vector<double> mgc((size_t)NM); std::vector<int> mtt((size_t)NM);
@@ -1674,8 +1674,6 @@
             max_batches[g] = std::max(max_batches[g], h_bbase[(size_t)g * (NC + 1) + i + 1] - h_bbase[(size_t)g * (NC + 1) + i]);
         bool segmented = stage == 0 && !use_wave && pga_dp_plan(chains.data(), NCH, tot_chain_nodes, seg_plan, seg_wave);
         if (seg_wave && !segmented) { seg_wave = false; wave_prep = use_wave; use_sched = false; h_bbase.clear(); }
-        const bool lean_gather = !P.want_nodes && !(getenv("PGA_TAIL") && strcmp(getenv("PGA_TAIL"), "host") == 0) && !getenv("PGA_FULL_GATHER");
-        const bool direct_gather = lean_gather && !getenv("PGA_GATHER_ALL_DP");
         const int64_t dp_cap = tot_chain_nodes + seg_plan.extra + 1;
         const int64_t dp_slots = NCH + (int64_t)seg_plan.segs.size() + 1;
         const int64_t tree_cap = use_wave ? 1 : (seg_wave ? tot_chain_nodes + 1 : dp_cap);
@@ -1794,6 +1792,7 @@
         tm.mark("plan+alloc");
         std::vector<int32_t> cs_tk[4], cs_en[4];
         ScoreParams sp{P.closed, P.meta, P.max_overlap, NM, nullptr, nullptr};
+        sp.lean_motifs = gene_only ? 1 : 0;
         PINBUF(h_conv, uint8_t, "h_conv_flag", (size_t)NG * NC + 1);
         const pga_training* d_models = (const pga_training*)c->d_models_raw;
         for (int g = 0; g < NG; g++) {
@@ -2275,7 +2274,7 @@
                 d.n = k >= 0 ? chains[k].n : 0; d.mx = k >= 0 ? h_maxidx[k] : -1;
                 d.st_wt = k >= 0 ? c->models[chains[k].model].st_wt : 0.0;
                 d.fin_off = k >= 0 ? fin_off[i] : 0; d.topo_off = k >= 0 ? chains[k].topo_off : 0;
-                d.group = k >= 0 ? chains[k].group : 0; d._pad = 0;
+                d.group = k >= 0 ? chains[k].group : 0; d.model = k >= 0 ? chains[k].model : 0;
                 d.dp_off = k >= 0 ? chains[k].off : 0;
                 n_slots += d.n / 2 + 2;
             }
@@ -2395,7 +2394,12 @@
                 GcPtrs gcs{};
                 for (int g = 0; g < NG; g++) gcs.p[g] = ga[g].gc_cont;
                 hipLaunchKernelGGL(k_emit_genes, dim3((unsigned)((n_slots + 255) / 256)), dim3(256), 0, st, d_td, NC, n_slots, o, d_gene2, d_ngenes,
-                                   d_gbegin, P.meta ? 0 : 1, d_genes, lean_gather ? 1 : 0, ca, gcs);
+                                   d_gbegin, P.meta ? 0 : 1, d_genes, lean_gather ? 1 : 0, ca, gcs, gene_only ? 1 : 0);
+                if (gene_only) {
+                    GeneTopo tp{};
+                    for (int g = 0; g < NG; g++) { tp.ndx[g] = ga[g].ndx; tp.stop_val[g] = ga[g].stop_val; tp.strand[g] = ga[g].strand; tp.edge0[g] = ga[g].edge0; }
+                    pga_launch_gene_fields(d_genes, ngenes, d_td, tp, d_ct, d_dig, total, d_models, f->d_sd_lut, st);
+                }
                 if (genes_out) HT(c, hipMemcpyAsync(genes_out, d_genes, sizeof(pga_gene) * (size_t)ngenes, hipMemcpyDeviceToHost, st));
                 if (keep) { keep->d_genes = d_genes; keep->n_genes = ngenes; }
             }
diff --git a/pyrodigal_amd/csrc/pipeline.h b/pyrodigal_amd/csrc/pipeline.h
--- a/pyrodigal_amd/csrc/pipeline.h
+++ b/pyrodigal_amd/csrc/pipeline.h
@@ -56,6 +56,7 @@
     unsigned long long* prof = nullptr;
     int32_t models_per_pass = 512;
     int32_t lean_stops = 0;
+    int32_t lean_motifs = 0;
 };
 
 void pga_launch_digitize(const char* d_seq, uint8_t* d_dig, int64_t total, const ContigDesc* d_ct, int n_contigs,
@@ -103,6 +104,19 @@
 int pga_extract_tile_size();
 void pga_launch_orf_gc(const ContigDesc* d_ct, int n_contigs, const uint8_t* d_dig, const int32_t* d_p16, const GroupArrays& ga,
                        int n_nodes_total, const int32_t* d_node_contig_base, hipStream_t st);
+struct TailDesc {
+    int64_t out_off;
+    int64_t gene_off;
+    int32_t n;
+    int32_t mx;
+    double  st_wt;
+    int64_t fin_off, topo_off;
+    int32_t group, model;
+    int64_t dp_off;
+};
+struct GeneTopo { const int32_t* ndx[4]; const int32_t* stop_val[4]; const int8_t* strand[4]; const uint8_t* edge0[4]; };
+void pga_launch_gene_fields(pga_gene* d_genes, int64_t n_genes, const TailDesc* d_td, const GeneTopo& topo, const ContigDesc* d_ct,
+                            const uint8_t* d_dig, int64_t total, const pga_training* d_models, const unsigned* d_sd_lut, hipStream_t st);
 void pga_launch_score(const ChainDesc* d_chains, int n_chains, int64_t node_begin, int64_t total, const uint8_t* d_dig,
                       const ContigDesc* d_ct, const GroupArrays& ga, const pga_training* d_models,
                       const ModelScoreConst* d_msc, const ModelConst* d_mc, const ChainArrays& ca, ScoreParams sp,
diff --git a/pyrodigal_amd/csrc/pipeline.hip b/pyrodigal_amd/csrc/pipeline.hip
--- a/pyrodigal_amd/csrc/pipeline.hip
+++ b/pyrodigal_amd/csrc/pipeline.hip
@@ -1576,6 +1576,64 @@
     return maxv;
 }
 
+template <int STEP>
+__device__ __forceinline__ void sd_search(const unsigned isA, const unsigned isG, const int start, const int strand, const unsigned* lut,
+                                          const double* rbs_wt, int& rbs0, int& rbs1, const int q0) {
+    constexpr int NQ = (15 + STEP - 1) / STEP;
+    unsigned pats[(NQ + 4) / 5] = {};
+#pragma unroll
+    for (int j = 0; j < NQ; j++) {
+        const int q = q0 + j * STEP;
+        if (STEP > 1 && q >= 15) continue;
+        const unsigned a6 = (isA >> (15 - q)) & 63u, g6 = (isG >> (15 - q)) & 63u;
+        const unsigned pat = ((a6 >> 5) & 1u) | (((g6 >> 4) & 1u) << 1) | (((g6 >> 3) & 1u) << 2) | (((a6 >> 2) & 1u) << 3) |
+                             (((g6 >> 1) & 1u) << 4) | ((g6 & 1u) << 5);
+        pats[j / 5] |= pat << (6 * (j % 5));
+    }
+#pragma unroll
+    for (int j = 0; j < NQ; j++) {
+        const int q = q0 + j * STEP;
+        if (STEP > 1 && q >= 15) continue;
+        if (start - 20 + q < 0 && strand == 1) continue;
+        const unsigned pat = (pats[j / 5] >> (6 * (j % 5))) & 63u;
+        const unsigned he = lut[(q << 6) | pat], hm = lut[((15 + q) << 6) | pat];
+        if (he > 1u) { const int a = sd_pick(he, rbs_wt); if (a > rbs0) rbs0 = a; }
+        if (hm > 1u) { const int b = sd_pick(hm, rbs_wt); if (b > rbs1) rbs1 = b; }
+    }
+}
+struct MotifBest { double score; int ndx, len, spacer, spacendx, order; };
+template <bool COMPACT, int STEP>
+__device__ __forceinline__ MotifBest motif_scan(const unsigned long long zm, const int start, const pga_training* __restrict__ tm,
+                                                const double* mk0, const double* mk1, const int t0) {
+    constexpr int NT = (13 + STEP - 1) / STEP;
+    auto midx = [&](const int k, const int t2) { return (int)((zm >> (2 * (21 - (18 + k - t2)))) & ((1ull << (2 * (k + 3))) - 1ull)); };
+    auto msi = [](const int t2) { return t2 <= 2 ? 3 : (t2 <= 4 ? 2 : (t2 >= 11 ? 1 : 0)); };
+    double bsc = -100.0; int bsp = 0, bsi = 0, blen = 0, bndx = 0, bord = 52;
+#pragma unroll 1
+    for (int k = 3; k >= 0; k--) {
+        const int stride = !COMPACT ? 4096 : (k == 0 ? 64 : (k == 1 ? 256 : 4096));
+        const double* __restrict__ gt = &tm->mot_wt[k][0][0];
+        const double* lt = k == 1 ? mk1 : mk0;
+        double scv[NT];
+        if (k >= 2 || !COMPACT) {
+#pragma unroll
+            for (int j = 0; j < NT; j++) { const int t2 = t0 + j * STEP; scv[j] = (t2 > 12 || 18 + k - t2 > start) ? -1000.0 : gt[msi(t2) * stride + midx(k, t2)]; }
+        } else {
+#pragma unroll
+            for (int j = 0; j < NT; j++) { const int t2 = t0 + j * STEP; scv[j] = (t2 > 12 || 18 + k - t2 > start) ? -1000.0 : lt[msi(t2) * stride + midx(k, t2)]; }
+        }
+#pragma unroll
+        for (int j = 0; j < NT; j++) {
+            const int t2 = t0 + j * STEP;
+            if (scv[j] > bsc) { bsc = scv[j]; bsi = msi(t2); bsp = 15 - t2; blen = k + 3; bndx = midx(k, t2); bord = 13 * (3 - k) + t2; }
+        }
+    }
+    return MotifBest{bsc, bndx, blen, bsp & 15, bsi, bord};
+}
+__device__ __forceinline__ void motif_keep(MotifBest& b, const double no_mot) {
+    if (b.score == -4.0 || b.score < no_mot + 0.69) b = MotifBest{no_mot, 0, 0, 0, 0, 0};
+}
+
 struct StartModel {
     double st_wt, no_mot;
     int tt, uses_sd;
@@ -2134,7 +2192,7 @@
     }
 }
 
-template <int TILE>
+template <int TILE, bool LEAN_MOTIFS >
 __global__ void __launch_bounds__(TILE, 8)
 k_score_starts_mm(const SsMmTile* __restrict__ tiles, const SsMmChain* __restrict__ mm, const SsStartRec* __restrict__ rec,
                   const pga_training* __restrict__ models, ChainArrays ca, ScoreParams sp, const unsigned* __restrict__ sd_lut) {
@@ -2201,8 +2259,6 @@
     int rbs0 = 0, rbs1 = 0, m_ndx = 0, m_len = 0, m_sp = 0, m_si = 0;
     double m_score = 0.0;
     const bool search_sd = !edge_in && SM.uses_sd, search_mot = !edge_in && !SM.uses_sd;
-    auto midx = [&](const int k, const int t2) { return (int)((zm >> (2 * (21 - (18 + k - t2)))) & ((1ull << (2 * (k + 3))) - 1ull)); };
-    auto msi = [](const int t2) { return t2 <= 2 ? 3 : (t2 <= 4 ? 2 : (t2 >= 11 ? 1 : 0)); };
     auto upstream = [&]() {
         double v = 0.0;
         unsigned lo32 = (unsigned)ucodes, hi32 = (unsigned)(ucodes >> 32);
@@ -2217,44 +2273,11 @@
         return v;
     };
     double u = 0.0;
-    if (search_sd) {
-        unsigned pats[3] = {0u, 0u, 0u};
-#pragma unroll
-        for (int q = 0; q < 15; q++) {
-            const unsigned a6 = (isA >> (15 - q)) & 63u, g6 = (isG >> (15 - q)) & 63u;
-            const unsigned pat = ((a6 >> 5) & 1u) | (((g6 >> 4) & 1u) << 1) | (((g6 >> 3) & 1u) << 2) | (((a6 >> 2) & 1u) << 3) |
-                                 (((g6 >> 1) & 1u) << 4) | ((g6 & 1u) << 5);
-            pats[q / 5] |= pat << (6 * (q % 5));
-        }
-#pragma unroll
-        for (int q = 0; q < 15; q++) {
-            if (start - 20 + q < 0 && strand == 1) continue;
-            const unsigned pat = (pats[q / 5] >> (6 * (q % 5))) & 63u;
-            const unsigned he = SM.lut[(q << 6) | pat], hm = SM.lut[((15 + q) << 6) | pat];
-            if (he > 1u) { const int a = sd_pick(he, SM.rbs_wt); if (a > rbs0) rbs0 = a; }
-            if (hm > 1u) { const int b = sd_pick(hm, SM.rbs_wt); if (b > rbs1) rbs1 = b; }
-        }
-    } else if (search_mot) {
-        double bsc = -100.0; int bsp = 0, bsi = 0, blen = 0, bndx = 0;
-#pragma unroll 1
-        for (int k = 3; k >= 0; k--) {
-            const int stride = k == 0 ? 64 : (k == 1 ? 256 : 4096);
-            const double* __restrict__ gt = &tm->mot_wt[k][0][0];
-            const double* lt = k == 1 ? &SM.mot.mk1[0][0] : &SM.mot.mk0[0][0];
-            double scv[13];
-            if (k >= 2) {
-#pragma unroll
-                for (int t2 = 0; t2 < 13; t2++) scv[t2] = 18 + k - t2 > start ? -1000.0 : gt[msi(t2) * stride + midx(k, t2)];
-            } else {
-#pragma unroll
-                for (int t2 = 0; t2 < 13; t2++) scv[t2] = 18 + k - t2 > start ? -1000.0 : lt[msi(t2) * stride + midx(k, t2)];
-            }
-#pragma unroll
-            for (int t2 = 0; t2 < 13; t2++)
-                if (scv[t2] > bsc) { bsc = scv[t2]; bsi = msi(t2); bsp = 15 - t2; blen = k + 3; bndx = midx(k, t2); }
-        }
-        if (bsc == -4.0 || bsc < SM.no_mot + 0.69) { m_score = SM.no_mot; }
-        else { m_ndx = bndx; m_len = blen; m_si = bsi; m_sp = bsp & 15; m_score = bsc; }
+    if (search_sd) sd_search<1>(isA, isG, start, strand, SM.lut, SM.rbs_wt, rbs0, rbs1, 0);
+    else if (search_mot) {
+        MotifBest h = motif_scan<true, 1>(zm, start, tm, &SM.mot.mk0[0][0], &SM.mot.mk1[0][0], 0);
+        motif_keep(h, SM.no_mot);
+        m_score = h.score; m_ndx = h.ndx; m_len = h.len; m_sp = h.spacer; m_si = h.spacendx;
     }
     if (!edge_in) u = upstream();
     mark(2);
@@ -2299,12 +2322,74 @@
     } else if (is_meta && cscore < 5.0 && orf < 120 && sscore < 0.0) sscore -= st_wt;
     mark(3);
     ca.cscore[g] = cscore; ca.sscore[g] = sscore; ca.rscore[g] = rscore; ca.uscore[g] = uscore; ca.tscore[g] = tscore;
-    ca.mot_score[g] = m_score; ca.mot_ndx[g] = m_ndx;
-    ca.mot_len[g] = (uint8_t)m_len; ca.mot_spacer[g] = (uint8_t)m_sp; ca.mot_spacendx[g] = (uint8_t)m_si;
-    ca.rbs[2 * g] = (uint8_t)rbs0; ca.rbs[2 * g + 1] = (uint8_t)rbs1;
+    if (!LEAN_MOTIFS) {
+        ca.mot_score[g] = m_score; ca.mot_ndx[g] = m_ndx;
+        ca.mot_len[g] = (uint8_t)m_len; ca.mot_spacer[g] = (uint8_t)m_sp; ca.mot_spacendx[g] = (uint8_t)m_si;
+        ca.rbs[2 * g] = (uint8_t)rbs0; ca.rbs[2 * g + 1] = (uint8_t)rbs1;
+    }
     ca.edge[g] = (uint8_t)edge_now;
     if (sp.cs_out != nullptr) sp.cs_out[g] = cscore + sscore;
     mark(4);
+    }
+}
+
+constexpr int GF_LANES = 4;
+__device__ __forceinline__ int gc_range_share(const uint8_t* __restrict__ dig, const int64_t a, const int64_t b, const int sub) {
+    const int64_t p0 = a & ~(int64_t)15;
+    int n = sub == 0 ? -gcn16(*reinterpret_cast<const uint4*>(dig + p0), (int)(a - p0)) : 0;
+    for (int64_t p = p0 + 16 * sub; p < b; p += 4 * 16 * GF_LANES) {
+        uint4 v[4];
+#pragma unroll
+        for (int j = 0; j < 4; j++) { const int64_t pj = p + j * 16 * GF_LANES; v[j] = *reinterpret_cast<const uint4*>(dig + (pj < b ? pj : p)); }
+#pragma unroll
+        for (int j = 0; j < 4; j++) n += gcn16(v[j], (int)max((int64_t)0, min((int64_t)16, b - (p + j * 16 * GF_LANES))));
+    }
+    return n;
+}
+__global__ void __launch_bounds__(256)
+k_gene_fields(pga_gene* __restrict__ genes, const int64_t n_genes, const TailDesc* __restrict__ td, const GeneTopo tp,
+              const ContigDesc* __restrict__ ct, const uint8_t* __restrict__ dig, const int64_t total,
+              const pga_training* __restrict__ models, const unsigned* __restrict__ sd_lut) {
+    const int64_t g = ((int64_t)blockIdx.x * blockDim.x + threadIdx.x) / GF_LANES;
+    const int sub = threadIdx.x % GF_LANES;
+    if (g >= n_genes) return;
+    const int c = genes[g].contig;
+    const int grp = td[c].group;
+    const int64_t ts = td[c].topo_off + genes[g].start_ndx;
+    const int ndx = tp.ndx[grp][ts], sv = tp.stop_val[grp][ts], strand = tp.strand[grp][ts];
+    const int L = ct[c].len;
+    const int64_t base = ct[c].base;
+    auto R = [&](const int x0, const int x1) { return gc_range_share(dig, max(base + x0, (int64_t)0), min(base + x1, total), sub); };
+    int cnt;
+    if (strand == 1) cnt = R(ndx, sv + 3);
+    else {
+        const int hi2 = min(ndx + 2, L - 1);
+        cnt = R(sv - 2, sv + 1) + (hi2 >= sv + 3 ? R(sv + 3, hi2 + 1) : 0);
+    }
+#pragma unroll
+    for (int m = GF_LANES / 2; m >= 1; m >>= 1) cnt += __shfl_xor(cnt, m, 64);
+    const double gsize = abs(sv - ndx) + 3.0;
+    if (sub == 0) genes[g].gc_cont = (float)((double)cnt / gsize);
+    if (tp.edge0[grp][ts]) return;
+    const pga_training* __restrict__ tm = &models[td[c].model];
+    const int start = strand == 1 ? ndx : L - 1 - ndx;
+    const UpWin W = load_upwin(dig + base, L, start, strand);
+    if (tm->uses_sd) {
+        int rbs0 = 0, rbs1 = 0;
+        sd_search<GF_LANES>(W.isA, W.isG, start, strand, sd_lut, tm->rbs_wt, rbs0, rbs1, sub);
+#pragma unroll
+        for (int m = GF_LANES / 2; m >= 1; m >>= 1) { rbs0 = max(rbs0, __shfl_xor(rbs0, m, 64)); rbs1 = max(rbs1, __shfl_xor(rbs1, m, 64)); }
+        if (sub == 0) { genes[g].rbs[0] = (uint8_t)rbs0; genes[g].rbs[1] = (uint8_t)rbs1; }
+    } else {
+        MotifBest h = motif_scan<false, GF_LANES>(W.zm & ((1ull << 42) - 1ull), start, tm, nullptr, nullptr, sub);
+#pragma unroll
+        for (int m = GF_LANES / 2; m >= 1; m >>= 1) {
+            const MotifBest o{__shfl_xor(h.score, m, 64), __shfl_xor(h.ndx, m, 64), __shfl_xor(h.len, m, 64), __shfl_xor(h.spacer, m, 64),
+                              __shfl_xor(h.spacendx, m, 64), __shfl_xor(h.order, m, 64)};
+            if (o.score > h.score || (o.score == h.score && o.order < h.order)) h = o;
+        }
+        motif_keep(h, tm->no_mot);
+        if (sub == 0) { genes[g].mot_score = h.score; genes[g].mot_ndx = h.ndx; genes[g].mot_len = (uint8_t)h.len; genes[g].mot_spacer = (uint8_t)h.spacer; }
     }
 }
 
@@ -2887,6 +2972,11 @@
                        n_nodes_total, d_node_contig_base);
 }
 
+void pga_launch_gene_fields(pga_gene* d_genes, int64_t n_genes, const TailDesc* d_td, const GeneTopo& topo, const ContigDesc* d_ct,
+                            const uint8_t* d_dig, int64_t total, const pga_training* d_models, const unsigned* d_sd_lut, hipStream_t st) {
+    if (n_genes <= 0) return;
+    hipLaunchKernelGGL(k_gene_fields, dim3(nblocks(n_genes * GF_LANES, 256)), dim3(256), 0, st, d_genes, n_genes, d_td, topo, d_ct, d_dig, total, d_models, d_sd_lut);
+}
 void pga_launch_sd_lut(unsigned* d_lut, hipStream_t st) {
     hipLaunchKernelGGL(k_sd_lut, dim3((PGA_SD_LUT + 255) / 256), dim3(256), 0, st, d_lut);
 }
@@ -2985,9 +3075,10 @@
             const SsMmTile* const d_tl = (const SsMmTile*)stops->mm_tile; const SsMmChain* const d_mc = (const SsMmChain*)stops->mm_chain;
             const SsStartRec* const d_rec = (const SsStartRec*)stops->mm_rec;
             const dim3 grid_mm((unsigned)stops->mm_tiles);
-            if (tile == 1024) hipLaunchKernelGGL(k_score_starts_mm<1024>, grid_mm, dim3(1024), 0, st, d_tl, d_mc, d_rec, d_models, ca, sp, d_sd_lut);
-            else if (tile == 512) hipLaunchKernelGGL(k_score_starts_mm<512>, grid_mm, dim3(512), 0, st, d_tl, d_mc, d_rec, d_models, ca, sp, d_sd_lut);
-            else hipLaunchKernelGGL(k_score_starts_mm<256>, grid_mm, blk, 0, st, d_tl, d_mc, d_rec, d_models, ca, sp, d_sd_lut);
+#define PGA_MM_LAUNCH(T, LEAN) hipLaunchKernelGGL((k_score_starts_mm<T, LEAN>), grid_mm, dim3(T), 0, st, d_tl, d_mc, d_rec, d_models, ca, sp, d_sd_lut)
+            if (sp.lean_motifs) { if (tile == 1024) PGA_MM_LAUNCH(1024, true); else if (tile == 512) PGA_MM_LAUNCH(512, true); else PGA_MM_LAUNCH(256, true); }
+            else { if (tile == 1024) PGA_MM_LAUNCH(1024, false); else if (tile == 512) PGA_MM_LAUNCH(512, false); else PGA_MM_LAUNCH(256, false); }
+#undef PGA_MM_LAUNCH
             if (stops->n_stops > 0)
                 hipLaunchKernelGGL(k_clear_stops, dim3(nblocks(stops->n_stops, 256)), blk, 0, st, d_all_chains, d_contig_chains, d_node_contig_base, ga, ca, sp,
                                    stops->n_stops);
```

Result: no change. 21060 Mbp/s (-0.5%).
